# Yukun-Huang/DreamWaltz-G

Measured on AMD Instinct MI355X. Metric: SDS steps/sec @512^2, 100k Gaussians, SD1.5+ControlNet; raster Mpix/s vs HBM roofline, higher is better.
Workload: dtype f32x

## Files before the change

### dreamwaltz-g_amd/csrc/gemm.hip

```cpp
#include "dwg_common.h"
#include "dwg_prof_internal.h"
#include "../../include/dwg_gemm.h"
#include <cstdlib>
#include <type_traits>

#if defined(DWG_GEMM_X_TU)
#include "dwg_xfmt.h"
typedef _Float16 HT;
#define DWG_DTYPE_HALF DWG_DTYPE_F32X
#define DWG_MFMA16(a, b, c) __builtin_amdgcn_mfma_f32_32x32x16_f16(a, b, c, 0, 0, 0)
#define DWG_HALF_NAME "f32x"
#elif defined(DWG_GEMM_F16_TU)
typedef _Float16 HT;
#define DWG_DTYPE_HALF DWG_DTYPE_F16
#define DWG_MFMA16(a, b, c) __builtin_amdgcn_mfma_f32_32x32x16_f16(a, b, c, 0, 0, 0)
#define DWG_HALF_NAME "f16"
#else
typedef __bf16 HT;
#define DWG_DTYPE_HALF DWG_DTYPE_BF16
#define DWG_MFMA16(a, b, c) __builtin_amdgcn_mfma_f32_32x32x16_bf16(a, b, c, 0, 0, 0)
#define DWG_HALF_NAME "bf16"
#endif

namespace {

typedef __attribute__((ext_vector_type(8))) HT bf16x8;
typedef __attribute__((ext_vector_type(16))) float f32x16;

struct ConvP {
    int enabled, Cin, Hin, Win, Hout, Wout, KH, KW, stride, pad_t, pad_l, dil;
    int up;
    int cin1;
    const void* A2;
};

struct GemmP {
    const void* A; const void* B; void* C; const void* bias; const void* residual;
    int M, N, K;
    long long sam, sak, sbn, sbk, ldc, ldr;
    int nb2;
    long long bA1, bA2, bB1, bB2, bC1, bC2, bR1, bR2;
    int act; float alpha;
    int out_bf16, res_bf16, bias_per_row, splitk, accumulate;
    float* ws;
    int bias_row_div;
    long long bias_ld;
    ConvP conv;
};

__device__ __forceinline__ float bf2f(HT x) { return (float)x; }
__device__ __forceinline__ HT f2bf(float x) { return (HT)x; }

struct bf16x4_t { HT v[4]; };
#ifdef DWG_GEMM_X_TU
__device__ __forceinline__ float ld_half1(const void* base, long long i) { return dwg_x_get1(base, i); }
__device__ __forceinline__ void st_half1(void* base, long long i, float v) { dwg_x_put1(base, i, v); }
__device__ __forceinline__ void ld_half4(const void* base, long long i, float (&v)[4]) { dwg_x_get4(base, i, v); }
__device__ __forceinline__ void st_half4(void* base, long long i, const float (&v)[4]) { dwg_x_put4(base, i, v); }
#else
__device__ __forceinline__ float ld_half1(const void* base, long long i) { return bf2f(reinterpret_cast<const HT*>(base)[i]); }
__device__ __forceinline__ void st_half1(void* base, long long i, float v) { reinterpret_cast<HT*>(base)[i] = f2bf(v); }
__device__ __forceinline__ void ld_half4(const void* base, long long i, float (&v)[4]) {
    const bf16x4_t r = *reinterpret_cast<const bf16x4_t*>(reinterpret_cast<const HT*>(base) + i);
#pragma unroll
    for (int e = 0; e < 4; e++) v[e] = bf2f(r.v[e]);
}
__device__ __forceinline__ void st_half4(void* base, long long i, const float (&v)[4]) {
    bf16x4_t o;
#pragma unroll
    for (int e = 0; e < 4; e++) o.v[e] = f2bf(v[e]);
    *reinterpret_cast<bf16x4_t*>(reinterpret_cast<HT*>(base) + i) = o;
}
#endif

template <bool LIGHT = false>
__device__ __forceinline__ float apply_act(float v, int act) {
    if constexpr (LIGHT) return act == 3 ? v / (1.f + __expf(-v)) : v;
    switch (act) {
        case 1: return v > 0.f ? v : 0.f;
        case 2: return v > 0.f ? v : 0.01f * v;
        case 3: return v / (1.f + __expf(-v));
        case 4: return 0.5f * v * (1.f + erff(v * 0.70710678118654752f));
        case 5: return 1.f / (1.f + __expf(-v));
        default: return v;
    }
}

template <typename T> struct TT;
template <> struct TT<HT> { static constexpr int VEC = 8; static constexpr int BK = 64; static constexpr int PAD = 8; };
template <> struct TT<float> { static constexpr int VEC = 4; static constexpr int BK = 16; static constexpr int PAD = 4; };

enum { MODE_KVEC = 0, MODE_RVEC = 1, MODE_SCALAR = 2, MODE_CONV = 3 };

template <typename T, int VEC> struct Chunk { T v[VEC]; };

template <typename T, int VEC>
__device__ __forceinline__ Chunk<T, VEC> load_vec(const T* p) {
    Chunk<T, VEC> c;
    *reinterpret_cast<uint4*>(&c) = *reinterpret_cast<const uint4*>(p);
    return c;
}
template <typename T, int VEC>
__device__ __forceinline__ Chunk<T, VEC> zero_chunk() {
    Chunk<T, VEC> c;
    *reinterpret_cast<uint4*>(&c) = make_uint4(0u, 0u, 0u, 0u);
    return c;
}

template <typename T, int ROWS, int MODE>
struct TileLoader {
    static constexpr int VEC = TT<T>::VEC, BK = TT<T>::BK, LDT = BK + TT<T>::PAD;
    static constexpr int CPR = BK / VEC, RPI = 256 / CPR;
    static constexpr int CPK = ROWS / VEC, KPI = 256 / CPK;
    static constexpr int NCH = (MODE == MODE_SCALAR) ? (ROWS * BK / 256) : (MODE == MODE_RVEC ? BK / KPI : ROWS / RPI);
    Chunk<T, VEC> regs[(MODE == MODE_SCALAR) ? 1 : NCH];
    T sregs[(MODE == MODE_SCALAR) ? NCH : 1];
    const T* rowptr[(MODE == MODE_KVEC) ? NCH : 1];
    int iy0[(MODE == MODE_CONV) ? NCH : 1], ix0[(MODE == MODE_CONV) ? NCH : 1];
    long long pix0[(MODE == MODE_CONV) ? NCH : 1];
    bool rok[(MODE == MODE_CONV) ? NCH : 1];
    const T* base; long long srow, sk; int nrows, r0, kcur, kend;
    int ci, ky, kx;

    __device__ __forceinline__ void init(const T* base_, long long srow_, long long sk_, int nrows_, int r0_, int kbeg, int kend_,
                                         const ConvP& cv) {
        base = base_; srow = srow_; sk = sk_; nrows = nrows_; r0 = r0_; kend = kend_;
        const int tid = threadIdx.x;
        if (MODE == MODE_KVEC) {
            kcur = kbeg + (tid % CPR) * VEC;
#pragma unroll
            for (int i = 0; i < NCH; i++) {
                int r = r0 + tid / CPR + i * RPI;
                rowptr[i] = r < nrows ? base + (long long)r * srow : nullptr;
            }
        } else if (MODE == MODE_CONV) {
            kcur = kbeg + (tid % CPR) * VEC;
            const int hw = cv.Hout * cv.Wout;
#pragma unroll
            for (int i = 0; i < NCH; i++) {
                int r = r0 + tid / CPR + i * RPI;
                rok[i] = r < nrows;
                int rr = rok[i] ? r : 0;
                int img = rr / hw, rem = rr - img * hw;
                int oy = rem / cv.Wout, ox = rem - oy * cv.Wout;
                iy0[i] = oy * cv.stride - cv.pad_t; ix0[i] = ox * cv.stride - cv.pad_l;
                pix0[i] = (long long)img * cv.Hin * cv.Win;
            }
            int tap = kcur / cv.Cin;
            ci = kcur - tap * cv.Cin; ky = tap / cv.KW; kx = tap - ky * cv.KW;
        } else {
            kcur = kbeg;
        }
    }

    __device__ __forceinline__ void advance(const ConvP& cv) {
        kcur += BK;
        if (MODE == MODE_CONV) {
            ci += BK;
            while (ci >= cv.Cin) { ci -= cv.Cin; if (++kx == cv.KW) { kx = 0; ++ky; } }
        }
    }

    __device__ __forceinline__ void load(const ConvP& cv) {
        const int tid = threadIdx.x;
        if (MODE == MODE_KVEC) {
            const bool kok = kcur < kend;
#pragma unroll
            for (int i = 0; i < NCH; i++)
                regs[i] = (kok && rowptr[i]) ? load_vec<T, VEC>(rowptr[i] + kcur) : zero_chunk<T, VEC>();
        } else if (MODE == MODE_CONV) {
            const bool kok = kcur < kend;
            const T* src0 = ci < cv.cin1 ? base : reinterpret_cast<const T*>(cv.A2);
            const int cs = ci < cv.cin1 ? cv.cin1 : (cv.Cin - cv.cin1);
            const int co = ci < cv.cin1 ? ci : ci - cv.cin1;
#pragma unroll
            for (int i = 0; i < NCH; i++) {
                int iy = iy0[i] + ky, ix = ix0[i] + kx;
                bool ok = kok && rok[i] && iy >= 0 && ix >= 0;
                if (cv.dil > 1) { ok = ok && (iy % cv.dil == 0) && (ix % cv.dil == 0); iy /= cv.dil; ix /= cv.dil; }
                if (cv.up > 1) { iy >>= 1; ix >>= 1; }
                ok = ok && iy < cv.Hin && ix < cv.Win;
                regs[i] = ok ? load_vec<T, VEC>(src0 + (pix0[i] + (long long)iy * cv.Win + ix) * cs + co) : zero_chunk<T, VEC>();
            }
        } else if (MODE == MODE_RVEC) {
#pragma unroll
            for (int i = 0; i < NCH; i++) {
                int kk = tid / CPK + i * KPI, rc = tid % CPK;
                int r = r0 + rc * VEC, k = kcur + kk;
                regs[i] = (r < nrows && k < kend) ? load_vec<T, VEC>(base + (long long)k * sk + r) : zero_chunk<T, VEC>();
            }
        } else {
#pragma unroll
            for (int i = 0; i < NCH; i++) {
                int c = tid + i * 256, row = c / BK, kk = c - row * BK;
                int r = r0 + row, k = kcur + kk;
                sregs[i] = (r < nrows && k < kend) ? base[(long long)r * srow + (long long)k * sk] : (T)0.f;
            }
        }
    }

    __device__ __forceinline__ void store(T* lds) {
        const int tid = threadIdx.x;
        if (MODE == MODE_KVEC || MODE == MODE_CONV) {
#pragma unroll
            for (int i = 0; i < NCH; i++)
                *reinterpret_cast<uint4*>(lds + (tid / CPR + i * RPI) * LDT + (tid % CPR) * VEC) = *reinterpret_cast<uint4*>(&regs[i]);
        } else if (MODE == MODE_RVEC) {
#pragma unroll
            for (int i = 0; i < NCH; i++) {
                int kk = tid / CPK + i * KPI, rc = tid % CPK;
#pragma unroll
                for (int e = 0; e < VEC; e++) lds[(rc * VEC + e) * LDT + kk] = regs[i].v[e];
            }
        } else {
#pragma unroll
            for (int i = 0; i < NCH; i++) {
                int c = tid + i * 256, row = c / BK, kk = c - row * BK;
                lds[row * LDT + kk] = sregs[i];
            }
        }
    }
};

template <typename T>
__device__ __forceinline__ void mma_tile(const T* sa, const T* sb, int lane, f32x16& acc);

template <>
__device__ __forceinline__ void mma_tile<HT>(const HT* sa, const HT* sb, int lane, f32x16& acc) {
    constexpr int LDT = TT<HT>::BK + TT<HT>::PAD;
    const HT* pa = sa + (lane & 31) * LDT + (lane >> 5) * 8;
    const HT* pb = sb + (lane & 31) * LDT + (lane >> 5) * 8;
#pragma unroll
    for (int ks = 0; ks < TT<HT>::BK / 16; ks++) {
        bf16x8 a = *reinterpret_cast<const bf16x8*>(pa + ks * 16);
        bf16x8 b = *reinterpret_cast<const bf16x8*>(pb + ks * 16);
        acc = DWG_MFMA16(a, b, acc);
    }
}
template <>
__device__ __forceinline__ void mma_tile<float>(const float* sa, const float* sb, int lane, f32x16& acc) {
    constexpr int LDT = TT<float>::BK + TT<float>::PAD;
    const float* pa = sa + (lane & 31) * LDT + (lane >> 5);
    const float* pb = sb + (lane & 31) * LDT + (lane >> 5);
#pragma unroll
    for (int ks = 0; ks < TT<float>::BK / 2; ks++)
        acc = __builtin_amdgcn_mfma_f32_32x32x2f32(pa[ks * 2], pb[ks * 2], acc, 0, 0, 0);
}

template <bool LIGHT = false>
__device__ __forceinline__ void epilogue_store(const GemmP& p, float v, int row, int col, long long coff, long long roff) {
    const long long ci = coff + (long long)row * p.ldc + col;
    if (p.bias) v += reinterpret_cast<const float*>(p.bias)[p.bias_row_div > 0 ? (long long)(row / p.bias_row_div) * p.bias_ld + col
                                                                             : (p.bias_per_row ? row : col)];
    v = apply_act<LIGHT>(v, p.act);
    if (p.residual) {
        const long long ri = roff + (long long)row * p.ldr + col;
        v += p.res_bf16 ? ld_half1(p.residual, ri) : reinterpret_cast<const float*>(p.residual)[ri];
    }
    if (p.out_bf16) st_half1(p.C, ci, v);
    else if (p.accumulate) reinterpret_cast<float*>(p.C)[ci] += v;
    else reinterpret_cast<float*>(p.C)[ci] = v;
}

__device__ __forceinline__ bool epilogue_vec_ok(const GemmP& p, long long coff, long long roff) {
    bool ok = (p.N & 3) == 0 && (p.ldc & 3) == 0 && (coff & 3) == 0 && ((uintptr_t)p.C & 15) == 0;
    if (p.residual) ok = ok && (p.ldr & 3) == 0 && (roff & 3) == 0 && ((uintptr_t)p.residual & 15) == 0;
    return ok;
}

template <bool LIGHT = false>
__device__ __forceinline__ void epilogue_store4(const GemmP& p, float (&v)[4], int row, int col, long long coff, long long roff, bool vec_ok) {
    if (!vec_ok || col + 3 >= p.N) {
#pragma unroll
        for (int e = 0; e < 4; e++)
            if (col + e < p.N) epilogue_store<LIGHT>(p, v[e], row, col + e, coff, roff);
        return;
    }
    if (p.bias) {
        const float* b = reinterpret_cast<const float*>(p.bias);
        if (p.bias_row_div > 0) {
            b += (long long)(row / p.bias_row_div) * p.bias_ld + col;
            v[0] += b[0]; v[1] += b[1]; v[2] += b[2]; v[3] += b[3];
        } else if (p.bias_per_row) {
            const float br = b[row];
            v[0] += br; v[1] += br; v[2] += br; v[3] += br;
        } else {
            v[0] += b[col]; v[1] += b[col + 1]; v[2] += b[col + 2]; v[3] += b[col + 3];
        }
    }
#pragma unroll
    for (int e = 0; e < 4; e++) v[e] = apply_act<LIGHT>(v[e], p.act);
    if (p.residual) {
        const long long ri = roff + (long long)row * p.ldr + col;
        if (p.res_bf16) {
            float r[4];
            ld_half4(p.residual, ri, r);
#pragma unroll
            for (int e = 0; e < 4; e++) v[e] += r[e];
        } else {
            float4 r = *reinterpret_cast<const float4*>(reinterpret_cast<const float*>(p.residual) + ri);
            v[0] += r.x; v[1] += r.y; v[2] += r.z; v[3] += r.w;
        }
    }
    const long long ci = coff + (long long)row * p.ldc + col;
    if (p.out_bf16) {
        st_half4(p.C, ci, v);
    } else {
        float4* dst = reinterpret_cast<float4*>(reinterpret_cast<float*>(p.C) + ci);
        float4 o = make_float4(v[0], v[1], v[2], v[3]);
        if (p.accumulate) { float4 c = *dst; o.x += c.x; o.y += c.y; o.z += c.z; o.w += c.w; }
        *dst = o;
    }
}

template <int BN, int BM = 128> struct EpiLds {
    static constexpr int LDC = BN + 4;
    static constexpr int passes(size_t lds_bytes) {
        return lds_bytes >= (size_t)BM * LDC * 4 ? 1 : (lds_bytes >= (size_t)(BM / 2) * LDC * 4 ? 2 : 4);
    }
    static constexpr size_t bytes(int npass) { return (size_t)(BM / npass) * LDC * 4; }
};

template <int BN, int NPASS, int TM, int TN, bool LIGHT, int BM = 128, int NT = 256, typename RowFn>
__device__ __forceinline__ void tile_epilogue_lds(const GemmP& p, f32x16 (&acc)[TM][TN], float* sC, int n0, int wm, int wn, int lane, int tid,
                                                  int ks_id, long long coff, long long roff, RowFn row_of) {
    constexpr int LDC = EpiLds<BN, BM>::LDC, C4 = BN / 4, PR = BM / NPASS;
    constexpr int BPP = BM / 32 / NPASS;
    static_assert(NT % C4 == 0 && (C4 & (C4 - 1)) == 0, "a thread keeps one column group");
    const bool vec_ok = epilogue_vec_ok(p, coff, roff);
    const int lrow = lane & 31, lhalf = (lane >> 5) * 4;
    const bool geglu = p.act == 6;
    const float* bias = reinterpret_cast<const float*>(p.bias);
    const bool fast = vec_ok && !geglu && !p.accumulate && !p.bias_per_row && (p.splitk <= 1 || p.ws) &&
                      (!bias || p.bias_row_div > 0 || ((uintptr_t)bias & 15) == 0) &&
                      (!bias || p.bias_row_div <= 0 || (((uintptr_t)bias & 15) == 0 && (p.bias_ld & 3) == 0)) &&
                      (p.splitk <= 1 || ((uintptr_t)p.ws & 15) == 0);
#pragma unroll 1
    for (int q = 0; q < NPASS; q++) {
        __syncthreads();
#pragma unroll
        for (int i = 0; i < TM; i++) {
            const int rb = wm * TM + i;
            if (NPASS > 1 && rb / BPP != q) continue;
            float* dst = sC + ((NPASS > 1 ? rb % BPP : rb) * 32 + lrow) * LDC + wn * 64 + lhalf;
#pragma unroll
            for (int j = 0; j < TN; j++)
#pragma unroll
                for (int r4 = 0; r4 < 4; r4++)
                    *reinterpret_cast<float4*>(dst + j * 32 + 8 * r4) =
                        make_float4(acc[i][j][4 * r4], acc[i][j][4 * r4 + 1], acc[i][j][4 * r4 + 2], acc[i][j][4 * r4 + 3]);
        }
        __syncthreads();
        if (geglu) {
            constexpr int G = C4 / 2, RSTEP = NT / G;
            const int o4 = tid & (G - 1), rl0 = tid / G;
            const int b = o4 >> 3, w = (o4 & 7) * 4;
            const int colp = n0 + b * 64 + w;
            if (colp + 35 < p.N) {
                float bh[4] = {0.f, 0.f, 0.f, 0.f}, bg[4] = {0.f, 0.f, 0.f, 0.f};
                if (bias) {
#pragma unroll
                    for (int e = 0; e < 4; e++) { bh[e] = bias[colp + e]; bg[e] = bias[colp + 32 + e]; }
                }
                const bool vec_store = ((p.ldc | coff) & 3) == 0 && ((uintptr_t)p.C & 7) == 0;
#pragma unroll 2
                for (int rl = rl0; rl < PR; rl += RSTEP) {
                    const int row = row_of(q * PR + rl);
                    if (row < 0) continue;
                    const float4 h = *reinterpret_cast<const float4*>(sC + rl * LDC + b * 64 + w);
                    const float4 g = *reinterpret_cast<const float4*>(sC + rl * LDC + b * 64 + 32 + w);
                    const float hv[4] = {h.x, h.y, h.z, h.w}, gv[4] = {g.x, g.y, g.z, g.w};
                    float v[4];
#pragma unroll
                    for (int e = 0; e < 4; e++) {
                        const float a = fmaf(hv[e], p.alpha, bh[e]);
                        const float gg = fmaf(gv[e], p.alpha, bg[e]);
                        v[e] = a * 0.5f * gg * (1.f + dwg_erf_fast(gg * 0.70710678118654752f));
                    }
                    const long long ci = coff + (long long)row * p.ldc + (n0 + b * 64) / 2 + w;
                    if (p.out_bf16) {
                        if (vec_store) {
                            st_half4(p.C, ci, v);
                        } else {
#pragma unroll
                            for (int e = 0; e < 4; e++) st_half1(p.C, ci + e, v[e]);
                        }
                    } else {
#pragma unroll
                        for (int e = 0; e < 4; e++) reinterpret_cast<float*>(p.C)[ci + e] = v[e];
                    }
                }
            }
            continue;
        }
        if (fast) {
            constexpr int RSTEP = NT / C4;
            const int c4 = tid & (C4 - 1), rl0 = tid / C4;
            const int col = n0 + c4 * 4;
            if (col < p.N) {
                const bool col_bias = bias && p.bias_row_div <= 0;
                float4 bc = make_float4(0.f, 0.f, 0.f, 0.f);
                if (col_bias) bc = *reinterpret_cast<const float4*>(bias + col);
                const bool slab = p.splitk > 1;
#pragma unroll 2
                for (int rl = rl0; rl < PR; rl += RSTEP) {
                    const int row = row_of(q * PR + rl);
                    if (row < 0) continue;
                    const float4 a = *reinterpret_cast<const float4*>(sC + rl * LDC + c4 * 4);
                    float v[4] = {a.x * p.alpha, a.y * p.alpha, a.z * p.alpha, a.w * p.alpha};
                    if (slab) {
                        *reinterpret_cast<float4*>(p.ws + ((long long)ks_id * p.M + row) * p.N + col) = make_float4(v[0], v[1], v[2], v[3]);
                        continue;
                    }
                    if (col_bias) { v[0] += bc.x; v[1] += bc.y; v[2] += bc.z; v[3] += bc.w; }
                    else if (bias) {
                        const float4 b = *reinterpret_cast<const float4*>(bias + (long long)(row / p.bias_row_div) * p.bias_ld + col);
                        v[0] += b.x; v[1] += b.y; v[2] += b.z; v[3] += b.w;
                    }
                    if (p.act == 3) {
#pragma unroll
                        for (int e = 0; e < 4; e++) v[e] = v[e] / (1.f + __expf(-v[e]));
                    } else if (p.act != 0) {
#pragma unroll
                        for (int e = 0; e < 4; e++) v[e] = apply_act<LIGHT>(v[e], p.act);
                    }
                    if (p.residual) {
                        const long long ri = roff + (long long)row * p.ldr + col;
                        if (p.res_bf16) {
                            float r[4];
                            ld_half4(p.residual, ri, r);
#pragma unroll
                            for (int e = 0; e < 4; e++) v[e] += r[e];
                        } else {
                            const float4 r = *reinterpret_cast<const float4*>(reinterpret_cast<const float*>(p.residual) + ri);
                            v[0] += r.x; v[1] += r.y; v[2] += r.z; v[3] += r.w;
                        }
                    }
                    const long long ci = coff + (long long)row * p.ldc + col;
                    if (p.out_bf16) {
                        st_half4(p.C, ci, v);
                    } else {
                        *reinterpret_cast<float4*>(reinterpret_cast<float*>(p.C) + ci) = make_float4(v[0], v[1], v[2], v[3]);
                    }
                }
            }
            continue;
        }
#pragma unroll 1
        for (int idx = tid; idx < PR * C4; idx += NT) {
            const int rl = idx / C4, c4 = idx - rl * C4;
            const int row = row_of(q * PR + rl), col = n0 + c4 * 4;
            if (row < 0 || col >= p.N) continue;
            const float4 a = *reinterpret_cast<const float4*>(sC + rl * LDC + c4 * 4);
            float v[4] = {a.x * p.alpha, a.y * p.alpha, a.z * p.alpha, a.w * p.alpha};
            if (p.splitk > 1) {
                if (p.ws) {
                    float* dst = p.ws + ((long long)ks_id * p.M + row) * p.N + col;
                    if ((p.N & 3) == 0) *reinterpret_cast<float4*>(dst) = make_float4(v[0], v[1], v[2], v[3]);
                    else {
#pragma unroll
                        for (int e = 0; e < 4; e++) if (col + e < p.N) dst[e] = v[e];
                    }
                } else {
#pragma unroll
                    for (int e = 0; e < 4; e++)
                        if (col + e < p.N) atomicAdd(reinterpret_cast<float*>(p.C) + coff + (long long)row * p.ldc + col + e, v[e]);
                }
                continue;
            }
            epilogue_store4<LIGHT>(p, v, row, col, coff, roff, vec_ok);
        }
    }
}

__global__ __launch_bounds__(256) void k_splitk_epilogue(GemmP p) {
    const long long n = (long long)p.M * p.N;
    if ((p.N & 3) == 0) {
        const bool vec_ok = epilogue_vec_ok(p, 0, 0);
        const int N4 = p.N >> 2;
        const long long n4 = n >> 2;
        for (long long i = (long long)blockIdx.x * 256 + threadIdx.x; i < n4; i += (long long)gridDim.x * 256) {
            const unsigned iu = (unsigned)i;
            const int row = (int)(iu / (unsigned)N4), col = (int)(iu - (unsigned)row * (unsigned)N4) * 4;
            const float4* src = reinterpret_cast<const float4*>(p.ws) + i;
            float4 a = src[0];
            int sidx = 1;
            for (; sidx + 3 < p.splitk; sidx += 4) {
                const float4 u0 = src[(long long)sidx * n4], u1 = src[(long long)(sidx + 1) * n4], u2 = src[(long long)(sidx + 2) * n4],
                             u3 = src[(long long)(sidx + 3) * n4];
                a.x += u0.x; a.y += u0.y; a.z += u0.z; a.w += u0.w;
                a.x += u1.x; a.y += u1.y; a.z += u1.z; a.w += u1.w;
                a.x += u2.x; a.y += u2.y; a.z += u2.z; a.w += u2.w;
                a.x += u3.x; a.y += u3.y; a.z += u3.z; a.w += u3.w;
            }
            if (sidx + 1 < p.splitk) {
                const float4 u0 = src[(long long)sidx * n4], u1 = src[(long long)(sidx + 1) * n4];
                a.x += u0.x; a.y += u0.y; a.z += u0.z; a.w += u0.w;
                a.x += u1.x; a.y += u1.y; a.z += u1.z; a.w += u1.w;
                sidx += 2;
            }
            if (sidx < p.splitk) {
                const float4 u = src[(long long)sidx * n4];
                a.x += u.x; a.y += u.y; a.z += u.z; a.w += u.w;
            }
            float v[4] = {a.x, a.y, a.z, a.w};
            epilogue_store4(p, v, row, col, 0, 0, vec_ok);
        }
        return;
    }
    for (long long i = (long long)blockIdx.x * 256 + threadIdx.x; i < n; i += (long long)gridDim.x * 256) {
        float v = 0.f;
        for (int s = 0; s < p.splitk; s++) v += p.ws[(long long)s * n + i];
        int row = (int)(i / p.N), col = (int)(i - (long long)row * p.N);
        epilogue_store(p, v, row, col, 0, 0);
    }
}

static void launch_splitk_epilogue(const GemmP& p, hipStream_t stream) {
    if (!(p.splitk > 1 && p.ws)) return;
    long long n = (long long)p.M * p.N;
    if ((p.N & 3) == 0) n >>= 2;
    int blocks = (int)((n + 255) / 256); if (blocks > 2048) blocks = 2048;
    DWG_LAUNCH("splitk_epilogue", k_splitk_epilogue, dim3(blocks), dim3(256), 0, stream, p);
}
template <typename T, int BN, int AMODE, int BMODE>
__global__ __launch_bounds__(256, (sizeof(T) == 4 || BN == 64) ? 2 : 1) void k_gemm(GemmP p) {
    constexpr int BM = 128, BK = TT<T>::BK, LDT = BK + TT<T>::PAD;
    constexpr int WN = BN / 64;
    constexpr int WM = 4 / WN;
    constexpr int TM = BM / WM / 32;
    constexpr int TN = 2;
    extern __shared__ __attribute__((aligned(16))) unsigned char smem_raw[];
    T* sA = reinterpret_cast<T*>(smem_raw);
    T* sB = sA + 2 * BM * LDT;
    const int tid = threadIdx.x, lane = tid & 63, wave = tid >> 6;
    const int wm = wave / WN, wn = wave % WN;
    const int m0 = blockIdx.x * BM;
    const int ntn = (p.N + BN - 1) / BN;
    const int n0 = (blockIdx.y % ntn) * BN;
    const int ks_id = blockIdx.y / ntn;
    const int z = blockIdx.z, z1 = z / p.nb2, z2 = z - z1 * p.nb2;
    const T* A = reinterpret_cast<const T*>(p.A) + z1 * p.bA1 + z2 * p.bA2;
    const T* B = reinterpret_cast<const T*>(p.B) + z1 * p.bB1 + z2 * p.bB2;
    int kbeg = 0, kend = p.K;
    if (p.splitk > 1) {
        int per = ((p.K + p.splitk - 1) / p.splitk + BK - 1) / BK * BK;
        kbeg = ks_id * per; kend = min(p.K, kbeg + per);
    }
    f32x16 acc[TM][TN];
#pragma unroll
    for (int i = 0; i < TM; i++)
#pragma unroll
        for (int j = 0; j < TN; j++)
#pragma unroll
            for (int r = 0; r < 16; r++) acc[i][j][r] = 0.f;

    TileLoader<T, BM, AMODE> la;
    TileLoader<T, BN, BMODE> lb;
    la.init(A, p.sam, p.sak, p.M, m0, kbeg, kend, p.conv);
    lb.init(B, p.sbn, p.sbk, p.N, n0, kbeg, kend, p.conv);
    const int nk = kend > kbeg ? (kend - kbeg + BK - 1) / BK : 0;
    if (nk > 0) {
        la.load(p.conv); lb.load(p.conv);
        la.store(sA); lb.store(sB);
    }
    __syncthreads();
    for (int kt = 0; kt < nk; kt++) {
        const int cur = kt & 1;
        if (kt + 1 < nk) {
            la.advance(p.conv); lb.advance(p.conv);
            la.load(p.conv); lb.load(p.conv);
        }
        const T* a = sA + cur * BM * LDT + (wm * TM * 32) * LDT;
        const T* b = sB + cur * BN * LDT + (wn * 64) * LDT;
#pragma unroll
        for (int i = 0; i < TM; i++)
#pragma unroll
            for (int j = 0; j < TN; j++) mma_tile<T>(b + j * 32 * LDT, a + i * 32 * LDT, lane, acc[i][j]);
        if (kt + 1 < nk) { la.store(sA + (cur ^ 1) * BM * LDT); lb.store(sB + (cur ^ 1) * BN * LDT); }
        __syncthreads();
    }
    constexpr int NPASS = EpiLds<BN>::passes((size_t)2 * (BM + BN) * LDT * sizeof(T));
    static_assert((size_t)2 * (BM + BN) * LDT * sizeof(T) >= EpiLds<BN>::bytes(NPASS), "epilogue staging fits in the operand stages");
    tile_epilogue_lds<BN, NPASS, TM, TN, false>(p, acc, reinterpret_cast<float*>(smem_raw), n0, wm, wn, lane, tid, ks_id, z1 * p.bC1 + z2 * p.bC2,
                                         z1 * p.bR1 + z2 * p.bR2, [&](int rl) { const int r = m0 + rl; return r < p.M ? r : -1; });
}

__device__ __attribute__((aligned(16))) unsigned char g_zero16[16];

template <int ROWS, bool CONV, int NW = 4>
struct GldsLoader {
    static constexpr int NJ = ROWS / (8 * NW);
    const HT* rowptr[CONV ? 1 : NJ];
    int iy0[CONV ? NJ : 1], ix0[CONV ? NJ : 1];
    long long pix0[CONV ? NJ : 1];
    bool rok[CONV ? NJ : 1];
    const HT* base;
    int kc[2], kend, ci[2], ky[2], kx[2];

    __device__ __forceinline__ void init(const HT* base_, long long srow, int nrows, int r0, int kbeg, int kend_, const ConvP& cv) {
        static_assert(NJ % 2 == 0, "row-block parity must equal j parity");
        base = base_; kend = kend_;
        const int lane = threadIdx.x & 63, wave = threadIdx.x >> 6, sub = lane >> 3;
        const int lg0 = (lane & 7) ^ (sub >> 1);
        kc[0] = kbeg + lg0 * 8; kc[1] = kbeg + (lg0 ^ 4) * 8;
        if (!CONV) {
#pragma unroll
            for (int j = 0; j < NJ; j++) {
                int r = r0 + (wave * NJ + j) * 8 + sub;
                rowptr[j] = r < nrows ? base + (long long)r * srow : nullptr;
            }
        } else {
            const int hw = cv.Hout * cv.Wout;
#pragma unroll
            for (int j = 0; j < NJ; j++) {
                int r = r0 + (wave * NJ + j) * 8 + sub;
                rok[j] = r < nrows;
                int rr = rok[j] ? r : 0;
                int img = rr / hw, rem = rr - img * hw;
                int oy = rem / cv.Wout, ox = rem - oy * cv.Wout;
                iy0[j] = oy * cv.stride - cv.pad_t; ix0[j] = ox * cv.stride - cv.pad_l;
                pix0[j] = (long long)img * cv.Hin * cv.Win;
            }
#pragma unroll
            for (int q = 0; q < 2; q++) {
                int tap = kc[q] / cv.Cin;
                ci[q] = kc[q] - tap * cv.Cin; ky[q] = tap / cv.KW; kx[q] = tap - ky[q] * cv.KW;
            }
        }
    }
    __device__ __forceinline__ void advance(const ConvP& cv) {
        kc[0] += 64; kc[1] += 64;
        if (CONV) {
#pragma unroll
            for (int q = 0; q < 2; q++) {
                ci[q] += 64;
                while (ci[q] >= cv.Cin) { ci[q] -= cv.Cin; if (++kx[q] == cv.KW) { kx[q] = 0; ++ky[q]; } }
            }
        }
    }
    __device__ __forceinline__ void issue(unsigned char* lds_tile, const ConvP& cv) {
        const int wave = __builtin_amdgcn_readfirstlane(threadIdx.x >> 6);
        const HT* zero = reinterpret_cast<const HT*>(g_zero16);
        const HT* src0[2] = {base, base}; int cs[2] = {0, 0}, co[2] = {0, 0};
        bool kok[2];
#pragma unroll
        for (int q = 0; q < 2; q++) {
            kok[q] = kc[q] < kend;
            if (CONV) {
                src0[q] = ci[q] < cv.cin1 ? base : reinterpret_cast<const HT*>(cv.A2);
                cs[q] = ci[q] < cv.cin1 ? cv.cin1 : (cv.Cin - cv.cin1);
                co[q] = ci[q] < cv.cin1 ? ci[q] : ci[q] - cv.cin1;
            }
        }
#pragma unroll
        for (int j = 0; j < NJ; j++) {
            const int q = j & 1;
            const HT* src;
            if (!CONV) {
                src = (kok[q] && rowptr[j]) ? rowptr[j] + kc[q] : zero;
            } else {
                int iy = iy0[j] + ky[q], ix = ix0[j] + kx[q];
                bool ok = kok[q] && rok[j] && iy >= 0 && ix >= 0;
                if (cv.dil > 1) { ok = ok && (iy % cv.dil == 0) && (ix % cv.dil == 0); iy /= cv.dil; ix /= cv.dil; }
                if (cv.up > 1) { iy >>= 1; ix >>= 1; }
                ok = ok && iy < cv.Hin && ix < cv.Win;
                src = ok ? src0[q] + (pix0[j] + (long long)iy * cv.Win + ix) * cs[q] + co[q] : zero;
            }
            unsigned char* dst = lds_tile + ((wave * NJ + j) * 8) * 128;
            __builtin_amdgcn_global_load_lds((const __attribute__((address_space(1))) void*)src,
                                             (__attribute__((address_space(3))) void*)dst, 16, 0, 0);
        }
    }
};

template <int ROWS, int NW = 4, bool CAT = false>
struct GldsConvFast {
    static constexpr int NJ = ROWS / (8 * NW);
    const unsigned char* pb[NJ];
    const unsigned char* pb2[CAT ? NJ : 1];
    unsigned int mask[NJ];
    int kcur, kend, tap, ci, ky, kx;

    __device__ __forceinline__ void init(const HT* base, long long, int nrows, int r0, int kbeg, int kend_, const ConvP& cv) {
        static_assert(NJ % 2 == 0, "row-block parity must equal j parity");
        const int lane = threadIdx.x & 63, wave = threadIdx.x >> 6, sub = lane >> 3;
        const int lg0 = (lane & 7) ^ (sub >> 1);
        kcur = kbeg; kend = kend_;
        tap = kbeg / cv.Cin; ci = kbeg - tap * cv.Cin; ky = tap / cv.KW; kx = tap - ky * cv.KW;
        const int hw = cv.Hout * cv.Wout;
        const int cs1 = CAT ? cv.cin1 : cv.Cin;
#pragma unroll
        for (int j = 0; j < NJ; j++) {
            const int r = r0 + (wave * NJ + j) * 8 + sub;
            const bool rok = r < nrows;
            const int rr = rok ? r : 0;
            const int img = rr / hw, rem = rr - img * hw;
            const int oy = rem / cv.Wout, ox = rem - oy * cv.Wout;
            const int iy0 = oy * cv.stride - cv.pad_t, ix0 = ox * cv.stride - cv.pad_l;
            unsigned int m = 0;
            for (int t = 0, y = 0; y < cv.KH; y++)
                for (int x = 0; x < cv.KW; x++, t++) {
                    const int iy = iy0 + y, ix = ix0 + x;
                    if (rok && iy >= 0 && iy < cv.Hin && ix >= 0 && ix < cv.Win) m |= 1u << t;
                }
            mask[j] = m;
            const long long pix = ((long long)img * cv.Hin + iy0) * cv.Win + ix0;
            pb[j] = reinterpret_cast<const unsigned char*>(base) + (pix * cs1 + (lg0 ^ ((j & 1) << 2)) * 8) * 2;
            if (CAT) pb2[j] = reinterpret_cast<const unsigned char*>(cv.A2) + (pix * (cv.Cin - cv.cin1) + (lg0 ^ ((j & 1) << 2)) * 8) * 2;
        }
    }
    __device__ __forceinline__ void advance(const ConvP& cv) {
        kcur += 64; ci += 64;
        const int w = ci >= cv.Cin ? 1 : 0;
        ci = w ? 0 : ci; tap += w; kx += w;
        const int w2 = kx == cv.KW ? 1 : 0;
        kx = w2 ? 0 : kx; ky += w2;
    }
    __device__ __forceinline__ void issue(unsigned char* lds_tile, const ConvP& cv) {
        const int wave = __builtin_amdgcn_readfirstlane(threadIdx.x >> 6);
        const unsigned char* zero = g_zero16;
        const bool second = CAT && ci >= cv.cin1;
        const int cs = CAT ? (second ? cv.Cin - cv.cin1 : cv.cin1) : cv.Cin;
        const long long uoff = (((long long)ky * cv.Win + kx) * cs + (second ? ci - cv.cin1 : ci)) * 2;
        const unsigned int bit = kcur < kend ? (1u << tap) : 0u;
#pragma unroll
        for (int j = 0; j < NJ; j++) {
            const unsigned char* src = (mask[j] & bit) ? ((CAT && second) ? pb2[j] : pb[j]) + uoff : zero;
            unsigned char* dst = lds_tile + ((wave * NJ + j) * 8) * 128;
            __builtin_amdgcn_global_load_lds((const __attribute__((address_space(1))) void*)src,
                                             (__attribute__((address_space(3))) void*)dst, 16, 0, 0);
        }
    }
};

template <int N>
__device__ __forceinline__ void wait_vmcnt() {
    __builtin_amdgcn_s_waitcnt((N & 15) | ((N >> 4) << 14) | (7 << 4) | (15 << 8));
}

template <int BM, int AKIND, int NW = 4> struct ALoaderOf { typedef GldsLoader<BM, false, NW> type; };
template <int BM, int NW> struct ALoaderOf<BM, 1, NW> { typedef GldsLoader<BM, true, NW> type; };
template <int BM, int NW> struct ALoaderOf<BM, 2, NW> { typedef GldsConvFast<BM, NW, false> type; };
template <int BM, int NW> struct ALoaderOf<BM, 3, NW> { typedef GldsConvFast<BM, NW, true> type; };

template <int BM, int BN> struct GldsGeom {
    static constexpr int WN = BN / 64, WM = (BM == 128 && BN == 64) ? 4 : BM / 64, NW = WM * WN, NT = NW * 64, TM = BM / WM / 32, TN = 2;
};

template <int BM, int BN, int AKIND, int S>
__device__ __forceinline__ void gemm_glds_body(const GemmP& p) {
    typedef GldsGeom<BM, BN> Geo;
    constexpr int WN = Geo::WN, WM = Geo::WM, NW = Geo::NW, NT = Geo::NT, TM = Geo::TM, TN = Geo::TN;
    constexpr int ABYTES = BM * 128, BBYTES = BN * 128, STAGE = ABYTES + BBYTES;
    extern __shared__ __attribute__((aligned(16))) unsigned char smem_raw[];
    const int tid = threadIdx.x, lane = tid & 63, wave = tid >> 6;
    const int wm = wave / WN, wn = wave % WN;
    const int gm = (p.M + BM - 1) / BM, ntn = (p.N + BN - 1) / BN;
    const int nwg = gridDim.x;
    int id = blockIdx.x;
    {
        const int q = nwg / 8, r = nwg % 8, xcd = id % 8, loc = id / 8;
        id = (xcd < r ? xcd * (q + 1) : r * (q + 1) + (xcd - r) * q) + loc;
    }
    const int tile = id % (gm * ntn), ks_id = id / (gm * ntn);
    const int m0 = (tile / ntn) * BM, n0 = (tile % ntn) * BN;
    const int z = blockIdx.z, z1 = z / p.nb2, z2 = z - z1 * p.nb2;
    const HT* A = reinterpret_cast<const HT*>(p.A) + z1 * p.bA1 + z2 * p.bA2;
    const HT* B = reinterpret_cast<const HT*>(p.B) + z1 * p.bB1 + z2 * p.bB2;
    int kbeg = 0, kend = p.K;
    if (p.splitk > 1) {
        int per = ((p.K + p.splitk - 1) / p.splitk + 63) / 64 * 64;
        kbeg = ks_id * per; kend = min(p.K, kbeg + per);
    }
    f32x16 acc[TM][TN];
#pragma unroll
    for (int i = 0; i < TM; i++)
#pragma unroll
        for (int j = 0; j < TN; j++)
#pragma unroll
            for (int r = 0; r < 16; r++) acc[i][j][r] = 0.f;
#ifdef DWG_GEMM_X_TU
    f32x16 acx[TM][TN];
#pragma unroll
    for (int i = 0; i < TM; i++)
#pragma unroll
        for (int j = 0; j < TN; j++)
#pragma unroll
            for (int r = 0; r < 16; r++) acx[i][j][r] = 0.f;
#endif
    typename ALoaderOf<BM, AKIND, NW>::type la;
    GldsLoader<BN, false, NW> lb;
    la.init(A, p.sam, p.M, m0, kbeg, kend, p.conv);
    lb.init(B, p.sbn, p.N, n0, kbeg, kend, p.conv);
    const int nk = kend > kbeg ? (kend - kbeg + 63) / 64 : 0;
    constexpr int LPT = (BM + BN) * 128 / (NT * 16);
#pragma unroll
    for (int s = 0; s < S - 1; s++) {
        la.issue(smem_raw + s * STAGE, p.conv); lb.issue(smem_raw + s * STAGE + ABYTES, p.conv);
        la.advance(p.conv); lb.advance(p.conv);
    }
    const int frow = lane & 31, fx = (lane >> 1) & 7, fh = lane >> 5;
#ifdef DWG_GEMM_X_TU
    constexpr int KS = 2;
    struct Frag { bf16x8 ah[TM], al[TM], bh[TN], bl[TN]; };
#else
    constexpr int KS = 4;
    struct Frag { bf16x8 af[TM], bf[TN]; };
#endif
    auto load_frags = [&](int stage, int ks, Frag& f) {
        const unsigned char* ta = smem_raw + stage * STAGE + (wm * TM * 32 + frow) * 128;
        const unsigned char* tb = smem_raw + stage * STAGE + ABYTES + (wn * 64 + frow) * 128;
#ifdef DWG_GEMM_X_TU
        const int offh = (((ks * 4 + fh * 2) ^ fx) << 4), offl = (((ks * 4 + fh * 2 + 1) ^ fx) << 4);
#pragma unroll
        for (int i = 0; i < TM; i++) {
            f.ah[i] = *reinterpret_cast<const bf16x8*>(ta + i * 32 * 128 + offh);
            f.al[i] = *reinterpret_cast<const bf16x8*>(ta + i * 32 * 128 + offl);
        }
#pragma unroll
        for (int j = 0; j < TN; j++) {
            f.bh[j] = *reinterpret_cast<const bf16x8*>(tb + j * 32 * 128 + offh);
            f.bl[j] = *reinterpret_cast<const bf16x8*>(tb + j * 32 * 128 + offl);
        }
#else
        const int off = (((ks * 2 + fh) ^ fx) << 4);
#pragma unroll
        for (int i = 0; i < TM; i++) f.af[i] = *reinterpret_cast<const bf16x8*>(ta + i * 32 * 128 + off);
#pragma unroll
        for (int j = 0; j < TN; j++) f.bf[j] = *reinterpret_cast<const bf16x8*>(tb + j * 32 * 128 + off);
#endif
    };
    auto mma = [&](const Frag& f) {
#ifdef DWG_GEMM_X_TU
#pragma unroll
        for (int i = 0; i < TM; i++)
#pragma unroll
            for (int j = 0; j < TN; j++) acc[i][j] = DWG_MFMA16(f.bh[j], f.ah[i], acc[i][j]);
#pragma unroll
        for (int i = 0; i < TM; i++)
#pragma unroll
            for (int j = 0; j < TN; j++) acx[i][j] = DWG_MFMA16(f.bl[j], f.ah[i], acx[i][j]);
#pragma unroll
        for (int i = 0; i < TM; i++)
#pragma unroll
            for (int j = 0; j < TN; j++) acx[i][j] = DWG_MFMA16(f.bh[j], f.al[i], acx[i][j]);
#else
#pragma unroll
        for (int i = 0; i < TM; i++)
#pragma unroll
            for (int j = 0; j < TN; j++) acc[i][j] = DWG_MFMA16(f.bf[j], f.af[i], acc[i][j]);
#endif
    };
    auto wait_tile_and_lds = [&]() {
        constexpr int N = (S - 2) * LPT;
        __builtin_amdgcn_s_waitcnt((N & 15) | ((N >> 4) << 14) | (7 << 4) | (0 << 8));
    };
    Frag F[2];
    int cur = 0, nxt = S - 1;
    if (nk > 0) {
        wait_vmcnt<(S - 2) * LPT>();
        __builtin_amdgcn_s_barrier();
        load_frags(0, 0, F[0]);
        __builtin_amdgcn_s_waitcnt(0xC07F);
    }
#ifdef DWG_GEMM_X_TU
    constexpr int MPS = 3 * TM * TN;
#else
    constexpr int MPS = TM * TN;
#endif
    for (int kt = 0; kt < nk; kt++) {
        const int cnext = cur + 1 == S ? 0 : cur + 1;
#pragma unroll
        for (int ks = 0; ks < KS; ks++) {
            if (ks + 1 < KS) {
                load_frags(cur, ks + 1, F[(ks + 1) & 1]);
            } else {
                wait_tile_and_lds();
                __builtin_amdgcn_s_barrier();
                load_frags(cnext, 0, F[0]);
            }
            __builtin_amdgcn_sched_barrier(0);
            if (ks == 0) {
                la.issue(smem_raw + nxt * STAGE, p.conv); lb.issue(smem_raw + nxt * STAGE + ABYTES, p.conv);
                la.advance(p.conv); lb.advance(p.conv);
            }
            mma(F[ks & 1]);
            if (ks == 0) {
#pragma unroll
                for (int m = 0; m < MPS; m++) {
                    __builtin_amdgcn_sched_group_barrier(0x008, 1, 0);
                    __builtin_amdgcn_sched_group_barrier(0x006, (LPT * 10 + MPS - 1) / MPS, 0);
                    __builtin_amdgcn_sched_group_barrier(0x020, (LPT + MPS - 1) / MPS, 0);
                }
            }
            __builtin_amdgcn_sched_barrier(0);
        }
        __builtin_amdgcn_s_waitcnt(0xC07F);
        cur = cnext; nxt = nxt + 1 == S ? 0 : nxt + 1;
    }
    wait_vmcnt<0>();
#ifdef DWG_GEMM_X_TU
#pragma unroll
    for (int i = 0; i < TM; i++)
#pragma unroll
        for (int j = 0; j < TN; j++)
#pragma unroll
            for (int r = 0; r < 16; r++) acc[i][j][r] = fmaf(acx[i][j][r], DWG_X_LO_INV, acc[i][j][r]);
#endif
    constexpr int NPASS = EpiLds<BN, BM>::passes((size_t)S * STAGE);
    static_assert((size_t)S * STAGE >= EpiLds<BN, BM>::bytes(NPASS), "epilogue staging fits in the operand stages");
    tile_epilogue_lds<BN, NPASS, TM, TN, false, BM, NT>(p, acc, reinterpret_cast<float*>(smem_raw), n0, wm, wn, lane, tid, ks_id, z1 * p.bC1 + z2 * p.bC2,
                                         z1 * p.bR1 + z2 * p.bR2, [&](int rl) { const int r = m0 + rl; return r < p.M ? r : -1; });
}

template <int BN, int AKIND, int S>
__global__ __launch_bounds__(256, 2) void k_gemm_glds(GemmP p) {
    gemm_glds_body<128, BN, AKIND, S>(p);
}

template <int BM, int BN, int AKIND, int S>
__global__ __launch_bounds__(512, 2) void k_gemm_glds8(GemmP p) {
    static_assert(GldsGeom<BM, BN>::NT == 512, "eight waves");
    gemm_glds_body<BM, BN, AKIND, S>(p);
}

static double gemm_flops(const GemmP& p, int batch) {
    double f = 2.0 * p.M * p.N * p.K * batch;
#ifdef DWG_GEMM_X_TU
    f *= 0.5;
#endif
    if (p.conv.enabled && p.conv.dil > 1) f /= (double)(p.conv.dil * p.conv.dil);
    return f;
}

template <int BN, int AKIND>
static void launch_glds(const GemmP& p, int batch, hipStream_t stream, const char* name) {
    constexpr int S = (BN == 64 && AKIND != 1) ? 3 : 2;
    size_t lds = (size_t)S * (128 + BN) * 128;
    static bool attr_set = false;
    if (!attr_set) {
        hipFuncSetAttribute(reinterpret_cast<const void*>(&k_gemm_glds<BN, AKIND, S>), hipFuncAttributeMaxDynamicSharedMemorySize, (int)lds);
        attr_set = true;
    }
    dim3 grid(((p.M + 127) / 128) * ((p.N + BN - 1) / BN) * (p.splitk > 1 ? p.splitk : 1), 1, batch);
    static const char* const sym[2][4] = {{"k_gemm_glds<64, 0, 3>", "k_gemm_glds<64, 1, 2>", "k_gemm_glds<64, 2, 3>", "k_gemm_glds<64, 3, 3>"},
                                          {"k_gemm_glds<128, 0, 2>", "k_gemm_glds<128, 1, 2>", "k_gemm_glds<128, 2, 2>", "k_gemm_glds<128, 3, 2>"}};
    DWG_LAUNCH_W(name, sym[BN == 128][AKIND], gemm_flops(p, batch), (k_gemm_glds<BN, AKIND, S>), grid, dim3(256), lds, stream, p);
    launch_splitk_epilogue(p, stream);
}

template <int BM, int BN, int AKIND>
static void launch_glds8(const GemmP& p, int batch, hipStream_t stream, const char* name) {
    constexpr int S = 3;
    const size_t lds = (size_t)S * (BM + BN) * 128;
    static bool attr_set = false;
    if (!attr_set) {
        hipFuncSetAttribute(reinterpret_cast<const void*>(&k_gemm_glds8<BM, BN, AKIND, S>), hipFuncAttributeMaxDynamicSharedMemorySize, (int)lds);
        attr_set = true;
    }
    dim3 grid(((p.M + BM - 1) / BM) * ((p.N + BN - 1) / BN) * (p.splitk > 1 ? p.splitk : 1), 1, batch);
    static const char* const sym[2][4] = {
        {"k_gemm_glds8<256, 128, 0, 3>", "k_gemm_glds8<256, 128, 1, 3>", "k_gemm_glds8<256, 128, 2, 3>", "k_gemm_glds8<256, 128, 3, 3>"},
        {"k_gemm_glds8<128, 256, 0, 3>", "k_gemm_glds8<128, 256, 1, 3>", "k_gemm_glds8<128, 256, 2, 3>", "k_gemm_glds8<128, 256, 3, 3>"}};
    DWG_LAUNCH_W(name, sym[BN == 256][AKIND], gemm_flops(p, batch), (k_gemm_glds8<BM, BN, AKIND, S>), grid, dim3(512), lds, stream, p);
    launch_splitk_epilogue(p, stream);
}

template <bool V> struct BoolC { static constexpr bool value = V; };
template <int BN, int NW> struct Patch2Geom {
    static constexpr int PH = NW == 8 ? 16 : 8, PW = 16, HP = PH + 2, WP = PW + 2, NPIX = HP * WP, BM = PH * PW;
    static constexpr int NPI = (NPIX + 7) / 8;
    static constexpr int PPW = (NPI + NW - 1) / NW;
    static constexpr int WN = BN / 64, WM = NW / WN, TM = BM / WM / 32, TN = 2, NT = NW * 64;
    static constexpr int NJW = BN / (8 * NW);
    static constexpr int PBYTES = NPI * 8 * 128, BBYTES = BN * 128;
};

template <int BN, bool SPLIT, int NW, int NBS>
__global__ __launch_bounds__(NW * 64, 2) void k_conv3x3_patch2(GemmP p) {
    typedef Patch2Geom<BN, NW> G;
    constexpr int PH = G::PH, PW = G::PW, WP = G::WP, NPIX = G::NPIX, NPI = G::NPI, PPW = G::PPW;
    constexpr int WN = G::WN, WM = G::WM, TM = G::TM, TN = G::TN, NT = G::NT, NJW = G::NJW, BM = G::BM;
    constexpr int PBYTES = G::PBYTES, BBYTES = G::BBYTES;
    static_assert(NJW >= 1 && (NJW % 2 == 0 || NJW == 1), "row-block parity");
    extern __shared__ __attribute__((aligned(16))) unsigned char smem_raw[];
    unsigned char* sP = smem_raw;
    unsigned char* sB = smem_raw + 2 * PBYTES;
    const ConvP& cv = p.conv;
    const int tid = threadIdx.x, lane = tid & 63, wave = tid >> 6;
    const int wv = __builtin_amdgcn_readfirstlane(wave);
    const int wm = wave / WN, wn = wave % WN;
    const int tiles_x = (cv.Wout + PW - 1) / PW, tiles_y = (cv.Hout + PH - 1) / PH;
    const int nimg = p.M / (cv.Hout * cv.Wout);
    const int gm = nimg * tiles_y * tiles_x, ntn = (p.N + BN - 1) / BN;
    int id = blockIdx.x;
    {
        const int nwg = gridDim.x, q = nwg / 8, r = nwg % 8, xcd = id % 8, loc = id / 8;
        id = (xcd < r ? xcd * (q + 1) : r * (q + 1) + (xcd - r) * q) + loc;
    }
    int ks_id = 0;
    if constexpr (SPLIT) { ks_id = id / (gm * ntn); id -= ks_id * gm * ntn; }
    const int mt = id / ntn, n0 = (id % ntn) * BN;
    const int img = mt / (tiles_y * tiles_x), trem = mt % (tiles_y * tiles_x);
    const int y0 = (trem / tiles_x) * PH, x0 = (trem % tiles_x) * PW;
    const HT* X = reinterpret_cast<const HT*>(p.A) + (long long)img * cv.Hin * cv.Win * cv.Cin;
    const HT* Wt = reinterpret_cast<const HT*>(p.B);
    const HT* zero = reinterpret_cast<const HT*>(g_zero16);
    const int sub = lane >> 3, lg0 = (lane & 7) ^ (sub >> 1);

    auto issue_patch = [&](int cc, bool valid, unsigned char* dst) {
#pragma unroll
        for (int q = 0; q < PPW; q++) {
            int inst = wv + q * NW;
            if (inst >= NPI) inst -= NW;
            const int pi = inst * 8 + sub;
            const int py = pi / WP, px = pi - py * WP;
            const int iy = y0 - 1 + py, ix = x0 - 1 + px;
            const bool ok = valid && pi < NPIX && iy >= 0 && iy < cv.Hin && ix >= 0 && ix < cv.Win;
            const HT* src = ok ? X + ((long long)iy * cv.Win + ix) * cv.Cin + (lg0 ^ ((inst & 1) << 2)) * 8 + cc * 64 : zero;
            __builtin_amdgcn_global_load_lds((const __attribute__((address_space(1))) void*)src,
                                             (__attribute__((address_space(3))) void*)(dst + inst * 8 * 128), 16, 0, 0);
        }
    };
    const HT* wrow[NJW];
#pragma unroll
    for (int j = 0; j < NJW; j++) {
        const int r = n0 + (wv * NJW + j) * 8 + sub;
        wrow[j] = r < p.N ? Wt + (long long)r * p.sbn + (lg0 ^ (((wv * NJW + j) & 1) << 2)) * 8 : nullptr;
    }
    auto issue_w = [&](int cc, int tap, bool valid, unsigned char* dst) {
        const long long kofs = (long long)tap * cv.Cin + cc * 64;
#pragma unroll
        for (int j = 0; j < NJW; j++) {
            const HT* src = (valid && wrow[j]) ? wrow[j] + kofs : zero;
            __builtin_amdgcn_global_load_lds((const __attribute__((address_space(1))) void*)src,
                                             (__attribute__((address_space(3))) void*)(dst + (wv * NJW + j) * 8 * 128), 16, 0, 0);
        }
    };
    f32x16 acc[TM][TN];
#pragma unroll
    for (int i = 0; i < TM; i++)
#pragma unroll
        for (int j = 0; j < TN; j++)
#pragma unroll
            for (int r = 0; r < 16; r++) acc[i][j][r] = 0.f;
#ifdef DWG_GEMM_X_TU
    f32x16 acx[TM][TN];
#pragma unroll
    for (int i = 0; i < TM; i++)
#pragma unroll
        for (int j = 0; j < TN; j++)
#pragma unroll
            for (int r = 0; r < 16; r++) acx[i][j][r] = 0.f;
    constexpr int KS = 2, MPS = 3 * TM * TN;
    struct Frag { bf16x8 ah[TM], al[TM], bh[TN], bl[TN]; };
#else
    constexpr int KS = 4, MPS = TM * TN;
    struct Frag { bf16x8 af[TM], bf[TN]; };
#endif
    int pbase[TM];
#pragma unroll
    for (int i = 0; i < TM; i++) {
        const int r = (wm * TM + i) * 32 + (lane & 31);
        pbase[i] = (r / PW) * WP + (r % PW);
    }
    int cc0 = 0, ncc = cv.Cin / 64;
    if constexpr (SPLIT) {
        const int per = (ncc + p.splitk - 1) / p.splitk;
        cc0 = ks_id * per; ncc = min(ncc, cc0 + per);
    }
    const int frow = lane & 31, fx = (lane >> 1) & 7, fh = lane >> 5;
    const int nsteps = max(0, ncc - cc0) * 9;
    auto load_frags = [&](const unsigned char* pa, int toff, const unsigned char* tbs, int ks, Frag& f) {
        const unsigned char* tb = tbs + (wn * 64 + frow) * 128;
#ifdef DWG_GEMM_X_TU
        const int cl = ks * 4 + fh * 2;
#pragma unroll
        for (int i = 0; i < TM; i++) {
            const int pi = pbase[i] + toff, sw = (pi >> 1) & 7;
            f.ah[i] = *reinterpret_cast<const bf16x8*>(pa + pi * 128 + ((cl ^ sw) << 4));
            f.al[i] = *reinterpret_cast<const bf16x8*>(pa + pi * 128 + (((cl + 1) ^ sw) << 4));
        }
#pragma unroll
        for (int j = 0; j < TN; j++) {
            f.bh[j] = *reinterpret_cast<const bf16x8*>(tb + j * 32 * 128 + ((cl ^ fx) << 4));
            f.bl[j] = *reinterpret_cast<const bf16x8*>(tb + j * 32 * 128 + (((cl + 1) ^ fx) << 4));
        }
#else
        const int cl = ks * 2 + fh;
#pragma unroll
        for (int i = 0; i < TM; i++) {
            const int pi = pbase[i] + toff;
            f.af[i] = *reinterpret_cast<const bf16x8*>(pa + pi * 128 + ((cl ^ ((pi >> 1) & 7)) << 4));
        }
#pragma unroll
        for (int j = 0; j < TN; j++) f.bf[j] = *reinterpret_cast<const bf16x8*>(tb + j * 32 * 128 + ((cl ^ fx) << 4));
#endif
    };
    auto mma = [&](const Frag& f) {
#ifdef DWG_GEMM_X_TU
#pragma unroll
        for (int i = 0; i < TM; i++)
#pragma unroll
            for (int j = 0; j < TN; j++) acc[i][j] = DWG_MFMA16(f.bh[j], f.ah[i], acc[i][j]);
#pragma unroll
        for (int i = 0; i < TM; i++)
#pragma unroll
            for (int j = 0; j < TN; j++) acx[i][j] = DWG_MFMA16(f.bl[j], f.ah[i], acx[i][j]);
#pragma unroll
        for (int i = 0; i < TM; i++)
#pragma unroll
            for (int j = 0; j < TN; j++) acx[i][j] = DWG_MFMA16(f.bh[j], f.al[i], acx[i][j]);
#else
#pragma unroll
        for (int i = 0; i < TM; i++)
#pragma unroll
            for (int j = 0; j < TN; j++) acc[i][j] = DWG_MFMA16(f.bf[j], f.af[i], acc[i][j]);
#endif
    };
    issue_patch(cc0, nsteps > 0, sP + (cc0 & 1) * PBYTES);
#pragma unroll
    for (int g = 0; g < NBS - 1; g++) issue_w(cc0 + g / 9, g % 9, g < nsteps, sB + g * BBYTES);
    Frag F[2];
    if (nsteps > 0) {
        wait_vmcnt<(NBS - 2) * NJW>();
        __builtin_amdgcn_s_barrier();
        load_frags(sP + (cc0 & 1) * PBYTES, 0, sB, 0, F[0]);
        __builtin_amdgcn_s_waitcnt(0xC07F);
    }
    int bst = 0;
    auto step = [&](auto is_tap0, int tap, int cc, const unsigned char* pa, const unsigned char* pan) {
        constexpr bool TAP0 = decltype(is_tap0)::value;
        const int ty = tap >= 6 ? 2 : (tap >= 3 ? 1 : 0);
        const int toff = ty * WP + (tap - 3 * ty);
        const int bnext = bst + 1 == NBS ? 0 : bst + 1;
        const int bfill = bst == 0 ? NBS - 1 : bst - 1;
        const unsigned char* tb = sB + bst * BBYTES;
#pragma unroll
        for (int ks = 0; ks < KS; ks++) {
            if (ks + 1 < KS) {
                load_frags(pa, toff, tb, ks + 1, F[(ks + 1) & 1]);
            } else {
                if (TAP0 || tap <= NBS - 2) {
                    constexpr int N = (NBS - 2) * NJW + PPW;
                    __builtin_amdgcn_s_waitcnt((N & 15) | ((N >> 4) << 14) | (7 << 4) | (0 << 8));
                } else {
                    constexpr int N = (NBS - 2) * NJW;
                    __builtin_amdgcn_s_waitcnt((N & 15) | ((N >> 4) << 14) | (7 << 4) | (0 << 8));
                }
                __builtin_amdgcn_s_barrier();
                const int ntap = tap == 8 ? 0 : tap + 1;
                const int nty = ntap >= 6 ? 2 : (ntap >= 3 ? 1 : 0);
                load_frags(tap == 8 ? pan : pa, nty * WP + (ntap - 3 * nty), sB + bnext * BBYTES, 0, F[0]);
            }
            __builtin_amdgcn_sched_barrier(0);
            if (ks == 0) {
                const int ft = tap + NBS - 1, fcc = cc + (ft >= 9 ? 1 : 0), ftap = ft >= 9 ? ft - 9 : ft;
                issue_w(fcc, ftap, fcc < ncc, sB + bfill * BBYTES);
                if (TAP0) issue_patch(cc + 1, cc + 1 < ncc, const_cast<unsigned char*>(pan));
            }
            mma(F[ks & 1]);
            if (ks == 0) {
                constexpr int NL = NJW + (TAP0 ? PPW : 0);
#pragma unroll
                for (int m = 0; m < MPS; m++) {
                    __builtin_amdgcn_sched_group_barrier(0x008, 1, 0);
                    __builtin_amdgcn_sched_group_barrier(0x006, (NL * 8 + MPS - 1) / MPS, 0);
                    __builtin_amdgcn_sched_group_barrier(0x020, (NL + MPS - 1) / MPS, 0);
                }
            }
            __builtin_amdgcn_sched_barrier(0);
        }
        __builtin_amdgcn_s_waitcnt(0xC07F);
        bst = bnext;
    };
    for (int cc = cc0; cc < ncc; cc++) {
        const unsigned char* pa = sP + (cc & 1) * PBYTES;
        const unsigned char* pan = sP + ((cc + 1) & 1) * PBYTES;
        step(BoolC<true>{}, 0, cc, pa, pan);
#pragma unroll 1
        for (int tap = 1; tap < 9; tap++) step(BoolC<false>{}, tap, cc, pa, pan);
    }
    wait_vmcnt<0>();
    __builtin_amdgcn_s_barrier();
#ifdef DWG_GEMM_X_TU
#pragma unroll
    for (int i = 0; i < TM; i++)
#pragma unroll
        for (int j = 0; j < TN; j++)
#pragma unroll
            for (int r = 0; r < 16; r++) acc[i][j][r] = fmaf(acx[i][j][r], DWG_X_LO_INV, acc[i][j][r]);
#endif
    constexpr int NPASS = EpiLds<BN, BM>::passes((size_t)2 * PBYTES + NBS * BBYTES);
    static_assert((size_t)2 * PBYTES + NBS * BBYTES >= EpiLds<BN, BM>::bytes(NPASS), "epilogue staging fits in the patch / weight buffers");
    tile_epilogue_lds<BN, NPASS, TM, TN, !SPLIT, BM, NT>(p, acc, reinterpret_cast<float*>(smem_raw), n0, wm, wn, lane, tid, ks_id, 0, 0, [&](int rr) {
        const int y = y0 + rr / PW, x = x0 + rr % PW;
        return (y < cv.Hout && x < cv.Wout) ? (img * cv.Hout + y) * cv.Wout + x : -1;
    });
}

template <int BN, int NW, int NBS>
static void launch_conv3x3_patch2(const GemmP& p, hipStream_t stream, const char* name) {
    typedef Patch2Geom<BN, NW> G;
    const size_t lds = (size_t)2 * G::PBYTES + (size_t)NBS * G::BBYTES;
    const ConvP& cv = p.conv;
    const int nimg = p.M / (cv.Hout * cv.Wout);
    const int gm = nimg * ((cv.Hout + G::PH - 1) / G::PH) * ((cv.Wout + G::PW - 1) / G::PW);
    dim3 grid(gm * ((p.N + BN - 1) / BN) * (p.splitk > 1 ? p.splitk : 1));
    static bool attr_set = false;
    if (!attr_set) {
        hipFuncSetAttribute(reinterpret_cast<const void*>(&k_conv3x3_patch2<BN, false, NW, NBS>), hipFuncAttributeMaxDynamicSharedMemorySize, (int)lds);
        hipFuncSetAttribute(reinterpret_cast<const void*>(&k_conv3x3_patch2<BN, true, NW, NBS>), hipFuncAttributeMaxDynamicSharedMemorySize, (int)lds);
        attr_set = true;
    }
    static_assert((NW == 8 && BN == 128 && NBS == 4) || (NW == 4 && BN == 64 && NBS == 4) || (NW == 4 && BN == 128 && NBS == 2), "symbol table below");
    const char* sym = NW == 8 ? (p.splitk > 1 && p.ws ? "k_conv3x3_patch2<128, true, 8, 4>" : "k_conv3x3_patch2<128, false, 8, 4>")
                              : (BN == 64 ? (p.splitk > 1 && p.ws ? "k_conv3x3_patch2<64, true, 4, 4>" : "k_conv3x3_patch2<64, false, 4, 4>")
                                          : (p.splitk > 1 && p.ws ? "k_conv3x3_patch2<128, true, 4, 2>" : "k_conv3x3_patch2<128, false, 4, 2>"));
    if (p.splitk > 1 && p.ws)
        DWG_LAUNCH_W(name, sym, gemm_flops(p, 1), (k_conv3x3_patch2<BN, true, NW, NBS>), grid, dim3(NW * 64), lds, stream, p);
    else
        DWG_LAUNCH_W(name, sym, gemm_flops(p, 1), (k_conv3x3_patch2<BN, false, NW, NBS>), grid, dim3(NW * 64), lds, stream, p);
    launch_splitk_epilogue(p, stream);
}

template <typename T, int BN, int AMODE, int BMODE>
static void launch(const GemmP& p, int batch, hipStream_t stream, const char* name) {
    constexpr int LDT = TT<T>::BK + TT<T>::PAD;
    size_t lds = (size_t)2 * (128 + BN) * LDT * sizeof(T);
    dim3 grid((p.M + 127) / 128, ((p.N + BN - 1) / BN) * (p.splitk > 1 ? p.splitk : 1), batch);
    static bool attr_set = false;
    if (!attr_set) {
        hipFuncSetAttribute(reinterpret_cast<const void*>(&k_gemm<T, BN, AMODE, BMODE>), hipFuncAttributeMaxDynamicSharedMemorySize,
                            (int)lds);
        attr_set = true;
    }
    DWG_LAUNCH_W(name, (sizeof(T) == 2 ? "k_gemm<" DWG_HALF_NAME ">" : "k_gemm<f32>"), gemm_flops(p, batch), (k_gemm<T, BN, AMODE, BMODE>), grid,
                 dim3(256), lds, stream, p);
    launch_splitk_epilogue(p, stream);
}

template <typename T, int BN, int AMODE>
static void dispatch_b(const GemmP& p, int bmode, int batch, hipStream_t s, const char* name) {
    if (bmode == MODE_KVEC) launch<T, BN, AMODE, MODE_KVEC>(p, batch, s, name);
    else if (bmode == MODE_RVEC) launch<T, BN, AMODE, MODE_RVEC>(p, batch, s, name);
    else launch<T, BN, AMODE, MODE_SCALAR>(p, batch, s, name);
}
template <typename T, int BN>
static void dispatch_a(const GemmP& p, int amode, int bmode, int batch, hipStream_t s, const char* name) {
    if (amode == MODE_KVEC) dispatch_b<T, BN, MODE_KVEC>(p, bmode, batch, s, name);
    else if (amode == MODE_RVEC) dispatch_b<T, BN, MODE_RVEC>(p, bmode, batch, s, name);
    else if (amode == MODE_CONV) dispatch_b<T, BN, MODE_CONV>(p, bmode, batch, s, name);
    else dispatch_b<T, BN, MODE_SCALAR>(p, bmode, batch, s, name);
}

static int batch_of(const dwg_gemm_desc* d) { return d->batch1 * d->batch2; }

static int tile_bn(const dwg_gemm_desc* d) {
    if (d->N <= 64) return 64;
    const long long blocks128 = (long long)((d->M + 127) / 128) * ((d->N + 127) / 128) * batch_of(d);
    return blocks128 < 256 ? 64 : 128;
}

constexpr int kCUs = 256, kMinWgs = 200;
static bool fills_cus(long long wgs) {
    const long long rounds = (wgs + kCUs - 1) / kCUs;
    return wgs >= kMinWgs && wgs * 100 >= rounds * kCUs * 80;
}

constexpr int kSplitkTarget = 256;
constexpr int kSplitkNoSplit = 384;
constexpr int kSplitkMinSteps = 12;
static int auto_splitk(int M, int N, int K, int bn, int bk) {
    long long blocks = (long long)((M + 127) / 128) * ((N + bn - 1) / bn);
    if (blocks >= kSplitkNoSplit || K < 2 * kSplitkMinSteps * bk) return 1;
    if (2.0 * M * N * K < 4.0e8) return 1;
    long long sk = kSplitkTarget / blocks;
    long long kmax = K / (kSplitkMinSteps * bk);
    if (sk > kmax) sk = kmax;
    if (sk > 16) sk = 16;
    return sk >= 2 ? (int)sk : 1;
}

constexpr int kBigMinK = 1280, kBigMaxTiles = 2048;
constexpr int kBigMinSteps = 8, kBigSkMax = 24;
static int big_tile(int M, int N, int K, int* splitk_out) {
    *splitk_out = 1;
    if (K < kBigMinK) return 0;
    int bm = 0;
    if (M >= 192) { if (N >= 128 && (N % 128 == 0 || N >= 640)) bm = 256; }
    else if (N >= 256) bm = 128;
    if (!bm) return 0;
    const int bn = bm == 256 ? 128 : 256;
    const long long tiles = (long long)((M + bm - 1) / bm) * ((N + bn - 1) / bn);
    if (tiles > kBigMaxTiles) return 0;
    long long sk = 1;
    if (tiles < kCUs) {
        sk = kCUs / tiles;
        const long long kmax = K / (kBigMinSteps * 64);
        if (sk > kmax) sk = kmax;
        if (sk > kBigSkMax) sk = kBigSkMax;
        if (sk < 1) sk = 1;
    }
    if (!fills_cus(tiles * sk)) return 0;
    *splitk_out = (int)sk;
    return bm;
}

template <typename T>
static int pick_mode(const void* base, long long srow, long long sk, int nrows, int K, const long long* boffs, int nboffs) {
    constexpr int VEC = TT<T>::VEC;
    bool aligned = ((uintptr_t)base % 16) == 0;
    for (int i = 0; i < nboffs; i++) aligned = aligned && (boffs[i] % VEC == 0);
    if (sk == 1 && aligned && K % VEC == 0 && srow % VEC == 0) return MODE_KVEC;
    if (srow == 1 && aligned && nrows % VEC == 0 && sk % VEC == 0) return MODE_RVEC;
    return MODE_SCALAR;
}

static int splitk_of(const dwg_gemm_desc* d) {
    if (d->splitk > 1) return d->splitk;
    if (d->splitk != 0 || d->act == DWG_ACT_GEGLU_PAIR) return 1;
    return auto_splitk(d->M, d->N, d->K, tile_bn(d), d->dtype == DWG_DTYPE_HALF ? TT<HT>::BK : TT<float>::BK);
}
static bool slabs_possible(const dwg_gemm_desc* d) { return batch_of(d) == 1 && (long long)d->M * d->N < (1LL << 33); }
static long long fit_workspace(const dwg_gemm_desc* d, long long sk) {
    while (sk > 1 && (size_t)sk * d->M * d->N * sizeof(float) > d->workspace_bytes) sk--;
    return sk;
}

enum Family { FAM_GENERIC, FAM_GLDS, FAM_GLDS8, FAM_PATCH2 };
struct Plan {
    Family fam;
    int bm, bn, nw;
    int amode, bmode;
    int akind;
    int splitk;
    bool slabs;
};

constexpr int kPatchMinM = 8192;
constexpr int kPatch8MinSteps = 100;

static int make_plan(const dwg_gemm_desc* d, const GemmP& p, Plan& pl) {
    const bool half = d->dtype == DWG_DTYPE_HALF;
#if defined(DWG_GEMM_F16_TU) || defined(DWG_GEMM_X_TU)
    if (!half) return DWG_E_ARG;
#endif
    pl = Plan{FAM_GENERIC, 128, tile_bn(d), 4, MODE_KVEC, MODE_KVEC, 0, d->splitk > 1 ? d->splitk : 1, false};
    if (d->workspace && slabs_possible(d)) {
        pl.splitk = (int)fit_workspace(d, splitk_of(d));
        pl.slabs = pl.splitk > 1;
    }
    const long long ao[2] = {p.bA1, p.bA2}, bo[2] = {p.bB1, p.bB2};
    if (p.conv.enabled) {
        const int vec = half ? TT<HT>::VEC : TT<float>::VEC;
        if (d->conv_cin % vec != 0 || ((uintptr_t)d->A % 16) != 0) return DWG_E_ARG;
        if (d->A2 && (d->conv_cin1 % vec != 0 || d->conv_cin1 <= 0 || d->conv_cin1 >= d->conv_cin || ((uintptr_t)d->A2 % 16) != 0))
            return DWG_E_ARG;
        if (d->K != d->conv_kh * d->conv_kw * d->conv_cin) return DWG_E_ARG;
        pl.amode = MODE_CONV;
    } else {
        pl.amode = half ? pick_mode<HT>(p.A, p.sam, p.sak, p.M, p.K, ao, 2) : pick_mode<float>(p.A, p.sam, p.sak, p.M, p.K, ao, 2);
    }
    pl.bmode = half ? pick_mode<HT>(p.B, p.sbn, p.sbk, p.N, p.K, bo, 2) : pick_mode<float>(p.B, p.sbn, p.sbk, p.N, p.K, bo, 2);
    if (!half) return DWG_OK;
    if (pl.bmode != MODE_KVEC || (pl.amode != MODE_KVEC && pl.amode != MODE_CONV)) {
#ifdef DWG_GEMM_X_TU
        return DWG_E_ARG;
#else
        return DWG_OK;
#endif
    }
    const ConvP& cv = p.conv;
    const char* minm = getenv("DWG_CONV_PATCH_MINM");
    const int patch_min_m = minm ? atoi(minm) : kPatchMinM;
    const bool patch_geom = pl.amode == MODE_CONV && batch_of(d) == 1 && d->conv_kh == 3 && d->conv_kw == 3 && d->conv_stride == 1 &&
                            cv.dil == 1 && cv.up == 1 && d->conv_pad_t == 1 && d->conv_pad_l == 1 && !d->A2 && d->conv_cin % 64 == 0 &&
                            d->conv_hout == d->conv_hin && d->conv_wout == d->conv_win && d->conv_wout >= 16 && d->conv_hout >= 8;
    const int ncc = d->conv_cin / 64;
    if (patch_geom && d->splitk <= 1 && d->conv_hout % 16 == 0 && d->conv_wout % 16 == 0 && (d->N % 128 == 0 || d->N >= 512)) {
        const long long tiles8 = (long long)(d->M / 256) * ((d->N + 127) / 128);
        long long sk = 1;
        if (tiles8 < kMinWgs && d->workspace && d->splitk == 0 && slabs_possible(d)) {
            sk = kCUs / tiles8;
            if (sk > ncc / 2) sk = ncc / 2;
            sk = fit_workspace(d, sk);
            if (sk < 1) sk = 1;
            const long long per = (ncc + sk - 1) / sk;
            sk = (ncc + per - 1) / per;
        }
        const long long steps = (ncc + sk - 1) / sk * 9;
        const bool worth = sk > 1 || steps >= kPatch8MinSteps || d->M < patch_min_m;
        if (worth && fills_cus(tiles8 * sk) && (d->act == 0 || d->act == 3 || sk > 1)) {
            pl = Plan{FAM_PATCH2, 256, 128, 8, MODE_CONV, pl.bmode, 0, (int)sk, sk > 1};
            return DWG_OK;
        }
    }
    if (patch_geom && d->M >= patch_min_m && (d->act == 0 || d->act == 3 || pl.splitk > 1)) {
        if (pl.splitk > 1) {
            const int gm = (d->M / (d->conv_hout * d->conv_wout)) * ((d->conv_hout + 7) / 8) * ((d->conv_wout + 15) / 16);
            const int blocks = gm * ((d->N + pl.bn - 1) / pl.bn);
            int sk = blocks >= 256 ? 1 : (384 + blocks - 1) / blocks;
            if (sk > ncc / 2) sk = ncc / 2;
            if (sk > pl.splitk) sk = pl.splitk;
            if (sk < 2) sk = 1;
            pl.splitk = sk;
            pl.slabs = pl.slabs && sk > 1;
        }
        pl.fam = FAM_PATCH2;
        return DWG_OK;
    }
    const bool fast_geom = pl.amode == MODE_CONV && d->conv_cin % 64 == 0 && cv.dil == 1 && cv.up == 1 && d->conv_kh * d->conv_kw <= 32;
    const bool cat_fast = d->A2 && d->conv_cin1 % 64 == 0 && (d->conv_cin - d->conv_cin1) % 64 == 0;
    pl.akind = pl.amode != MODE_CONV ? 0 : (fast_geom && !d->A2 ? 2 : (fast_geom && cat_fast ? 3 : 1));
    int big_sk = 1;
    const int big_bm = d->splitk <= 1 ? big_tile(d->M, d->N, d->K, &big_sk) : 0;
    if (big_bm) {
        if (d->act == DWG_ACT_GEGLU_PAIR || !d->workspace || !slabs_possible(d) || d->splitk == 1) big_sk = 1;
        big_sk = (int)fit_workspace(d, big_sk);
        const int bbn = big_bm == 256 ? 128 : 256;
        const long long tiles = (long long)((d->M + big_bm - 1) / big_bm) * ((d->N + bbn - 1) / bbn) * batch_of(d);
        if (fills_cus(tiles * big_sk)) {
            pl = Plan{FAM_GLDS8, big_bm, bbn, 8, pl.amode, pl.bmode, pl.akind, big_sk, big_sk > 1};
            return DWG_OK;
        }
    }
    pl.fam = FAM_GLDS;
    return DWG_OK;
}

template <typename T>
static void launch_generic(const GemmP& p, const Plan& pl, int batch, hipStream_t s, const char* name) {
    if (pl.bn == 64) dispatch_a<T, 64>(p, pl.amode, pl.bmode, batch, s, name);
    else dispatch_a<T, 128>(p, pl.amode, pl.bmode, batch, s, name);
}
template <typename F>
static void with_akind(int akind, F f) {
    if (akind == 3) f(std::integral_constant<int, 3>{});
    else if (akind == 2) f(std::integral_constant<int, 2>{});
    else if (akind == 1) f(std::integral_constant<int, 1>{});
    else f(std::integral_constant<int, 0>{});
}

}

#ifdef DWG_GEMM_X_TU
static bool x_physical(const dwg_gemm_desc* d, dwg_gemm_desc* o) {
    if (!d) return false;
    *o = *d;
    if (d->dtype != DWG_DTYPE_F32X) return false;
    if (d->K % 8 || d->a_k_stride != 1 || d->b_k_stride != 1) return false;
    if ((d->a_row_stride | d->b_row_stride | d->a_batch1_stride | d->a_batch2_stride | d->b_batch1_stride | d->b_batch2_stride) % 8) return false;
    if (d->out_dtype == DWG_DTYPE_F32X && ((d->ldc | d->c_batch1_stride | d->c_batch2_stride) % 8 || ((uintptr_t)d->C % 16))) return false;
    if (d->residual && d->residual_dtype == DWG_DTYPE_F32X &&
        (((d->ldr ? d->ldr : d->ldc) | d->r_batch1_stride | d->r_batch2_stride) % 8 || ((uintptr_t)d->residual % 16))) return false;
    if (d->act == DWG_ACT_GEGLU_PAIR && d->out_dtype == DWG_DTYPE_F32X && d->N % 16) return false;
    if (d->conv_enabled && (d->conv_cin % 8 || (d->A2 && d->conv_cin1 % 8))) return false;
    o->K = 2 * d->K;
    o->a_row_stride = 2 * d->a_row_stride; o->b_row_stride = 2 * d->b_row_stride;
    o->a_batch1_stride = 2 * d->a_batch1_stride; o->a_batch2_stride = 2 * d->a_batch2_stride;
    o->b_batch1_stride = 2 * d->b_batch1_stride; o->b_batch2_stride = 2 * d->b_batch2_stride;
    o->conv_cin = 2 * d->conv_cin; o->conv_cin1 = 2 * d->conv_cin1;
    return true;
}
#endif

extern "C" {

#if defined(DWG_GEMM_X_TU)
#define DWG_GEMM_FN dwg_gemm_x
#define DWG_GEMM_WS_FN dwg_gemm_workspace_bytes_x
#elif defined(DWG_GEMM_F16_TU)
#define DWG_GEMM_FN dwg_gemm_f16
#define DWG_GEMM_WS_FN dwg_gemm_workspace_bytes_f16
#else
#define DWG_GEMM_FN dwg_gemm
#define DWG_GEMM_WS_FN dwg_gemm_workspace_bytes
size_t dwg_gemm_workspace_bytes_f16(const dwg_gemm_desc* d);
int dwg_gemm_f16(const dwg_gemm_desc* d, dwg_stream_t stream);
size_t dwg_gemm_workspace_bytes_x(const dwg_gemm_desc* d);
int dwg_gemm_x(const dwg_gemm_desc* d, dwg_stream_t stream);
#endif

size_t DWG_GEMM_WS_FN(const dwg_gemm_desc* d) {
#if !defined(DWG_GEMM_F16_TU) && !defined(DWG_GEMM_X_TU)
    if (d && d->dtype == DWG_DTYPE_F16) return dwg_gemm_workspace_bytes_f16(d);
    if (d && d->dtype == DWG_DTYPE_F32X) return dwg_gemm_workspace_bytes_x(d);
#endif
#ifdef DWG_GEMM_X_TU
    dwg_gemm_desc xd;
    if (!x_physical(d, &xd)) return 0;
    d = &xd;
#endif
    if (!d || d->M <= 0 || d->N <= 0 || !slabs_possible(d)) return 0;
    dwg_gemm_desc pd = *d;
    if (d->plan_m > d->M) pd.M = d->plan_m;
    d = &pd;
    int sk = splitk_of(d);
    if (d->dtype == DWG_DTYPE_HALF && d->splitk == 0 && d->act != DWG_ACT_GEGLU_PAIR) {
        int bsk = 1;
        if (big_tile(d->M, d->N, d->K, &bsk) && bsk > sk) sk = bsk;
    }
    return sk > 1 ? (size_t)sk * d->M * d->N * sizeof(float) : 0;
}

int DWG_GEMM_FN(const dwg_gemm_desc* d, dwg_stream_t stream_) {
#if !defined(DWG_GEMM_F16_TU) && !defined(DWG_GEMM_X_TU)
    if (d && d->dtype == DWG_DTYPE_F16) return dwg_gemm_f16(d, stream_);
    if (d && d->dtype == DWG_DTYPE_F32X) return dwg_gemm_x(d, stream_);
#endif
#ifdef DWG_GEMM_X_TU
    dwg_gemm_desc xd;
    if (!x_physical(d, &xd)) return DWG_E_ARG;
    d = &xd;
#endif
    if (!d || !d->A || !d->B || !d->C) return DWG_E_ARG;
    if (d->M < 0 || d->N < 0 || d->K < 0 || d->batch1 < 1 || d->batch2 < 1 || d->plan_m < 0) return DWG_E_ARG;
    if (d->M == 0 || d->N == 0) return DWG_OK;
    if (d->dtype != DWG_DTYPE_F32 && d->dtype != DWG_DTYPE_HALF) return DWG_E_ARG;
    if (d->splitk > 1 && !d->workspace && (d->out_dtype != DWG_DTYPE_F32 || d->bias || d->residual || d->act)) return DWG_E_ARG;
    if (d->accumulate && d->out_dtype != DWG_DTYPE_F32) return DWG_E_ARG;
    if (d->act == DWG_ACT_GEGLU_PAIR && (d->N % 64 != 0 || d->residual || d->splitk > 1 || d->bias_per_row || d->bias_row_div)) return DWG_E_ARG;
    if ((uintptr_t)d->workspace & 15) return DWG_E_ARG;
    GemmP p;
    p.A = d->A; p.B = d->B; p.C = d->C; p.bias = d->bias; p.residual = d->residual;
    p.M = d->M; p.N = d->N; p.K = d->K;
    p.sam = d->a_row_stride; p.sak = d->a_k_stride; p.sbn = d->b_row_stride; p.sbk = d->b_k_stride;
    p.ldc = d->ldc; p.ldr = d->ldr ? d->ldr : d->ldc;
    p.nb2 = d->batch2;
    p.bA1 = d->a_batch1_stride; p.bA2 = d->a_batch2_stride; p.bB1 = d->b_batch1_stride; p.bB2 = d->b_batch2_stride;
    p.bC1 = d->c_batch1_stride; p.bC2 = d->c_batch2_stride; p.bR1 = d->r_batch1_stride; p.bR2 = d->r_batch2_stride;
    p.act = d->act; p.alpha = d->alpha;
    p.out_bf16 = d->out_dtype == DWG_DTYPE_HALF; p.res_bf16 = d->residual_dtype == DWG_DTYPE_HALF;
    p.bias_per_row = d->bias_per_row; p.accumulate = d->accumulate;
    const bool plain1x1 = d->conv_enabled && d->conv_kh == 1 && d->conv_kw == 1 && d->conv_stride == 1 && d->conv_pad_t == 0 &&
                          d->conv_pad_l == 0 && d->conv_in_dilation <= 1 && d->conv_in_upsample <= 1 && !d->A2 && d->conv_hout == d->conv_hin &&
                          d->conv_wout == d->conv_win && d->K == d->conv_cin && batch_of(d) == 1;
    if (plain1x1) { p.sam = d->conv_cin; p.sak = 1; }
    p.conv.enabled = d->conv_enabled && !plain1x1;
    p.conv.Cin = d->conv_cin; p.conv.Hin = d->conv_hin; p.conv.Win = d->conv_win; p.conv.Hout = d->conv_hout;
    p.conv.Wout = d->conv_wout; p.conv.KH = d->conv_kh; p.conv.KW = d->conv_kw; p.conv.stride = d->conv_stride;
    p.conv.pad_t = d->conv_pad_t; p.conv.pad_l = d->conv_pad_l; p.conv.dil = d->conv_in_dilation > 1 ? d->conv_in_dilation : 1;
    p.conv.up = d->conv_in_upsample > 1 ? d->conv_in_upsample : 1;
    p.conv.A2 = d->A2; p.conv.cin1 = d->A2 ? d->conv_cin1 : d->conv_cin;
    p.bias_row_div = d->bias_row_div; p.bias_ld = d->bias_ld > 0 ? d->bias_ld : d->N;
    Plan pl;
    dwg_gemm_desc pd = *d;
    if (d->plan_m > d->M) pd.M = d->plan_m;
    const int rc = make_plan(&pd, p, pl);
    if (rc != DWG_OK) return rc;
    p.splitk = pl.splitk;
    p.ws = pl.slabs ? reinterpret_cast<float*>(d->workspace) : nullptr;
    const int batch = batch_of(d);
    hipStream_t stream = (hipStream_t)stream_;
    const char* name = d->name ? d->name : (d->conv_enabled ? "conv_igemm" : "gemm");
    switch (pl.fam) {
        case FAM_PATCH2:
            if (pl.nw == 8) launch_conv3x3_patch2<128, 8, 4>(p, stream, name);
            else if (pl.bn == 64) launch_conv3x3_patch2<64, 4, 4>(p, stream, name);
            else launch_conv3x3_patch2<128, 4, 2>(p, stream, name);
            break;
        case FAM_GLDS8:
            with_akind(pl.akind, [&](auto ak) {
                if (pl.bm == 256) launch_glds8<256, 128, decltype(ak)::value>(p, batch, stream, name);
                else launch_glds8<128, 256, decltype(ak)::value>(p, batch, stream, name);
            });
            break;
        case FAM_GLDS:
            with_akind(pl.akind, [&](auto ak) {
                if (pl.bn == 64) launch_glds<64, decltype(ak)::value>(p, batch, stream, name);
                else launch_glds<128, decltype(ak)::value>(p, batch, stream, name);
            });
            break;
        case FAM_GENERIC:
#if defined(DWG_GEMM_X_TU)
            return DWG_E_ARG;
#elif defined(DWG_GEMM_F16_TU)
            launch_generic<HT>(p, pl, batch, stream, name);
#else
            if (d->dtype == DWG_DTYPE_HALF) launch_generic<HT>(p, pl, batch, stream, name);
            else launch_generic<float>(p, pl, batch, stream, name);
#endif
            break;
    }
    DWG_RETURN_IF_LAUNCH_FAILED();
    return DWG_OK;
}

}
```

### dreamwaltz-g_amd/gemm.py

```python
import ctypes

import torch

from . import _lib

F32, BF16, F16, F32X = 0, 1, 2, 3
ACT = {None: 0, "none": 0, "relu": 1, "leaky_relu": 2, "silu": 3, "gelu": 4, "sigmoid": 5, "geglu_pair": 6}


class GemmDesc(ctypes.Structure):
    _fields_ = [
        ("A", ctypes.c_void_p), ("B", ctypes.c_void_p), ("C", ctypes.c_void_p), ("bias", ctypes.c_void_p),
        ("residual", ctypes.c_void_p),
        ("M", ctypes.c_int32), ("N", ctypes.c_int32), ("K", ctypes.c_int32),
        ("a_row_stride", ctypes.c_int64), ("a_k_stride", ctypes.c_int64), ("b_row_stride", ctypes.c_int64),
        ("b_k_stride", ctypes.c_int64), ("ldc", ctypes.c_int64), ("ldr", ctypes.c_int64),
        ("batch1", ctypes.c_int32), ("batch2", ctypes.c_int32),
        ("a_batch1_stride", ctypes.c_int64), ("a_batch2_stride", ctypes.c_int64), ("b_batch1_stride", ctypes.c_int64),
        ("b_batch2_stride", ctypes.c_int64), ("c_batch1_stride", ctypes.c_int64), ("c_batch2_stride", ctypes.c_int64),
        ("r_batch1_stride", ctypes.c_int64), ("r_batch2_stride", ctypes.c_int64),
        ("dtype", ctypes.c_int32), ("out_dtype", ctypes.c_int32), ("residual_dtype", ctypes.c_int32),
        ("act", ctypes.c_int32), ("alpha", ctypes.c_float), ("bias_per_row", ctypes.c_int32),
        ("splitk", ctypes.c_int32), ("accumulate", ctypes.c_int32),
        ("conv_enabled", ctypes.c_int32), ("conv_cin", ctypes.c_int32), ("conv_hin", ctypes.c_int32),
        ("conv_win", ctypes.c_int32), ("conv_hout", ctypes.c_int32), ("conv_wout", ctypes.c_int32),
        ("conv_kh", ctypes.c_int32), ("conv_kw", ctypes.c_int32), ("conv_stride", ctypes.c_int32),
        ("conv_pad_t", ctypes.c_int32), ("conv_pad_l", ctypes.c_int32), ("conv_in_dilation", ctypes.c_int32),
        ("conv_in_upsample", ctypes.c_int32), ("A2", ctypes.c_void_p), ("conv_cin1", ctypes.c_int32),
        ("bias_row_div", ctypes.c_int32), ("bias_ld", ctypes.c_int64),
        ("workspace", ctypes.c_void_p), ("workspace_bytes", ctypes.c_size_t),
        ("name", ctypes.c_char_p), ("plan_m", ctypes.c_int32),
    ]


def _dt(t):
    if t.dtype == torch.float32:
        return F32
    if t.dtype == torch.bfloat16:
        return BF16
    if t.dtype == torch.float16:
        return F16
    if t.dtype == torch.int32:
        return F32X
    raise TypeError("dwg gemm supports float32, bfloat16, float16 and f32x (int32-typed, xfmt.py) tensors, got %s" % t.dtype)


def _stream(t):
    return ctypes.c_void_p(torch.cuda.current_stream(t.device).cuda_stream)


def gemm_raw(A, B, C, M, N, K, a_strides, b_strides, ldc, bias=None, residual=None, ldr=0, act=None, alpha=1.0,
             batch=(1, 1), a_batch=(0, 0), b_batch=(0, 0), c_batch=(0, 0), r_batch=(0, 0), bias_per_row=False, splitk=1,
             accumulate=False, conv=None, name=None, conv_upsample=1, A2=None, cin1=0, bias_row_div=0, bias_ld=0, plan_m=0, run=True):
    if not A.is_cuda:
        raise RuntimeError("dreamwaltz_g_amd GEMM runs on the GPU only (HIP kernels)")
    d = GemmDesc()
    d.A, d.B, d.C = A.data_ptr(), B.data_ptr(), C.data_ptr()
    d.bias = bias.data_ptr() if bias is not None else None
    d.residual = residual.data_ptr() if residual is not None else None
    d.M, d.N, d.K = M, N, K
    d.a_row_stride, d.a_k_stride = a_strides
    d.b_row_stride, d.b_k_stride = b_strides
    d.ldc, d.ldr = ldc, ldr
    d.batch1, d.batch2 = batch
    d.a_batch1_stride, d.a_batch2_stride = a_batch
    d.b_batch1_stride, d.b_batch2_stride = b_batch
    d.c_batch1_stride, d.c_batch2_stride = c_batch
    d.r_batch1_stride, d.r_batch2_stride = r_batch
    d.dtype = _dt(A)
    assert _dt(B) == d.dtype, "A and B must share a dtype"
    d.out_dtype = _dt(C)
    d.residual_dtype = _dt(residual) if residual is not None else F32
    d.act = ACT[act]
    d.alpha = alpha
    d.bias_per_row = int(bias_per_row)
    d.splitk = splitk
    d.accumulate = int(accumulate)
    if conv is not None:
        d.conv_enabled = 1
        (d.conv_cin, d.conv_hin, d.conv_win, d.conv_hout, d.conv_wout, d.conv_kh, d.conv_kw, d.conv_stride, d.conv_pad_t,
         d.conv_pad_l, d.conv_in_dilation) = conv
    d.conv_in_upsample = conv_upsample
    if A2 is not None:
        d.A2 = A2.data_ptr(); d.conv_cin1 = cin1
    d.bias_row_div = bias_row_div
    d.bias_ld = bias_ld
    d.name = name.encode() if name else None
    d.plan_m = plan_m
    if not run:
        return d
    _lib.check(_lib.lib().dwg_gemm(ctypes.byref(d), _stream(A)), "dwg_gemm")
    return C


def run_desc(d, stream):
    rc = _lib.lib().dwg_gemm(ctypes.byref(d), stream)
    if rc != 0:
        raise RuntimeError("dwg_gemm failed with DWG error %d" % rc)


def linear(x, w, bias=None, act=None, out_dtype=None, residual=None, out=None, name=None):
    K = x.shape[-1]
    x2 = x.reshape(-1, K)
    M, N = x2.shape[0], w.shape[0]
    out_dtype = out_dtype or x.dtype
    y = out if out is not None else torch.empty(M, N, device=x.device, dtype=out_dtype)
    r2 = None if residual is None else residual.reshape(M, N)
    gemm_raw(x2, w, y, M, N, K, (x2.stride(0), x2.stride(1)), (w.stride(0), w.stride(1)), y.stride(0), bias=bias, residual=r2,
             ldr=0 if r2 is None else r2.stride(0), act=act, name=name)
    return y.reshape(*x.shape[:-1], N)


def conv2d_nhwc(x, w, bias=None, stride=1, pad=(1, 1), act=None, residual=None, out_hw=None, in_dilation=1, out_dtype=None,
                name=None):
    Bn, H, W, Cin = x.shape
    Cout, KH, KW, _ = w.shape
    Hv, Wv = (H - 1) * in_dilation + 1, (W - 1) * in_dilation + 1
    if out_hw is None:
        Ho = (Hv + 2 * pad[0] - KH) // stride + 1
        Wo = (Wv + 2 * pad[1] - KW) // stride + 1
    else:
        Ho, Wo = out_hw
    y = torch.empty(Bn, Ho, Wo, Cout, device=x.device, dtype=out_dtype or x.dtype)
    M, N, K = Bn * Ho * Wo, Cout, KH * KW * Cin
    gemm_raw(x, w, y, M, N, K, (0, 1), (K, 1), Cout, bias=bias, residual=residual, ldr=Cout if residual is not None else 0,
             act=act, conv=(Cin, H, W, Ho, Wo, KH, KW, stride, pad[0], pad[1], in_dilation), name=name)
    return y
```

### dreamwaltz-g_amd/sd15.py

```python
import ctypes
import os
import math
from collections import OrderedDict
from dataclasses import dataclass
from typing import Dict, List, Optional, Tuple

import torch

from . import _lib, gemm, xfmt

BF16 = torch.bfloat16

TORCH_DTYPE = {"bf16": torch.bfloat16, "f32": torch.float32, "f16": torch.float16, "f32x": xfmt.DTYPE}
DT_CODE = {"f32": 0, "bf16": 1, "f16": 2, "f32x": 3}


def dtype_name(dtype) -> str:
    names = {"bf16": "bf16", "bfloat16": "bf16", torch.bfloat16: "bf16", "f32": "f32", "fp32": "f32", "float32": "f32", torch.float32: "f32",
             "f16": "f16", "fp16": "f16", "float16": "f16", "half": "f16", torch.float16: "f16", "f32x": "f32x", "fp32x": "f32x"}
    if dtype not in names:
        raise ValueError("plan dtype must be one of bf16 / f32 / f16 / f32x, got %r" % (dtype,))
    return names[dtype]


@dataclass
class UNetConfig:
    in_channels: int = 4
    out_channels: int = 4
    block_out_channels: Tuple[int, ...] = (320, 640, 1280, 1280)
    layers_per_block: int = 2
    heads: int = 8
    cross_dim: int = 768
    groups: int = 32
    attn_blocks: Tuple[bool, ...] = (True, True, True, False)
    cond_channels: Tuple[int, ...] = (16, 32, 96, 256)
    cond_in_channels: int = 3

    @property
    def temb_dim(self):
        return self.block_out_channels[0] * 4


@dataclass
class VAEConfig:
    in_channels: int = 3
    block_out_channels: Tuple[int, ...] = (128, 256, 512, 512)
    layers_per_block: int = 2
    latent_channels: int = 4
    groups: int = 32
    scaling_factor: float = 0.18215


def _cfg_get(config, key, default):
    if config is None:
        return default
    if isinstance(config, dict):
        return config.get(key, default)
    return getattr(config, key, default)


def unet_config_from(config) -> "UNetConfig":
    d = UNetConfig()
    if config is None:
        return d
    boc = tuple(int(c) for c in _cfg_get(config, "block_out_channels", d.block_out_channels))
    down = tuple(_cfg_get(config, "down_block_types", ("CrossAttnDownBlock2D",) * 3 + ("DownBlock2D",)))
    heads = _cfg_get(config, "attention_head_dim", d.heads)
    if isinstance(heads, (list, tuple)):
        if len(set(heads)) != 1:
            raise NotImplementedError("per-level attention_head_dim %r (SDXL-style UNets are outside this path)" % (heads,))
        heads = heads[0]
    for key, want in (("transformer_layers_per_block", 1), ("class_embed_type", None), ("addition_embed_type", None), ("use_linear_projection", False),
                      ("only_cross_attention", False), ("dual_cross_attention", False)):
        got = _cfg_get(config, key, want)
        if got != want:
            raise NotImplementedError("UNet config %s=%r (SD-1.x layer graph only)" % (key, got))
    return UNetConfig(in_channels=int(_cfg_get(config, "in_channels", d.in_channels)), out_channels=int(_cfg_get(config, "out_channels", d.out_channels)),
                      block_out_channels=boc, layers_per_block=int(_cfg_get(config, "layers_per_block", d.layers_per_block)), heads=int(heads),
                      cross_dim=int(_cfg_get(config, "cross_attention_dim", d.cross_dim)), groups=int(_cfg_get(config, "norm_num_groups", d.groups)),
                      attn_blocks=tuple(t.startswith("CrossAttn") for t in down))


def vae_config_from(config) -> "VAEConfig":
    d = VAEConfig()
    if config is None:
        return d
    return VAEConfig(in_channels=int(_cfg_get(config, "in_channels", d.in_channels)),
                     block_out_channels=tuple(int(c) for c in _cfg_get(config, "block_out_channels", d.block_out_channels)),
                     layers_per_block=int(_cfg_get(config, "layers_per_block", d.layers_per_block)),
                     latent_channels=int(_cfg_get(config, "latent_channels", d.latent_channels)), groups=int(_cfg_get(config, "norm_num_groups", d.groups)),
                     scaling_factor=float(_cfg_get(config, "scaling_factor", d.scaling_factor)))


def _resnet_shapes(sh, pre, cin, cout, temb):
    sh[pre + ".norm1.weight"] = (cin,); sh[pre + ".norm1.bias"] = (cin,)
    sh[pre + ".conv1.weight"] = (cout, cin, 3, 3); sh[pre + ".conv1.bias"] = (cout,)
    if temb:
        sh[pre + ".time_emb_proj.weight"] = (cout, temb); sh[pre + ".time_emb_proj.bias"] = (cout,)
    sh[pre + ".norm2.weight"] = (cout,); sh[pre + ".norm2.bias"] = (cout,)
    sh[pre + ".conv2.weight"] = (cout, cout, 3, 3); sh[pre + ".conv2.bias"] = (cout,)
    if cin != cout:
        sh[pre + ".conv_shortcut.weight"] = (cout, cin, 1, 1); sh[pre + ".conv_shortcut.bias"] = (cout,)


def _transformer_shapes(sh, pre, c, cross):
    sh[pre + ".norm.weight"] = (c,); sh[pre + ".norm.bias"] = (c,)
    sh[pre + ".proj_in.weight"] = (c, c, 1, 1); sh[pre + ".proj_in.bias"] = (c,)
    t = pre + ".transformer_blocks.0"
    for n in ("norm1", "norm2", "norm3"):
        sh["%s.%s.weight" % (t, n)] = (c,); sh["%s.%s.bias" % (t, n)] = (c,)
    for a, kd in (("attn1", c), ("attn2", cross)):
        sh["%s.%s.to_q.weight" % (t, a)] = (c, c)
        sh["%s.%s.to_k.weight" % (t, a)] = (c, kd)
        sh["%s.%s.to_v.weight" % (t, a)] = (c, kd)
        sh["%s.%s.to_out.0.weight" % (t, a)] = (c, c); sh["%s.%s.to_out.0.bias" % (t, a)] = (c,)
    sh[t + ".ff.net.0.proj.weight"] = (8 * c, c); sh[t + ".ff.net.0.proj.bias"] = (8 * c,)
    sh[t + ".ff.net.2.weight"] = (c, 4 * c); sh[t + ".ff.net.2.bias"] = (c,)
    sh[pre + ".proj_out.weight"] = (c, c, 1, 1); sh[pre + ".proj_out.bias"] = (c,)


def _encoder_shapes(sh, cfg: UNetConfig):
    boc = cfg.block_out_channels
    sh["conv_in.weight"] = (boc[0], cfg.in_channels, 3, 3); sh["conv_in.bias"] = (boc[0],)
    sh["time_embedding.linear_1.weight"] = (cfg.temb_dim, boc[0]); sh["time_embedding.linear_1.bias"] = (cfg.temb_dim,)
    sh["time_embedding.linear_2.weight"] = (cfg.temb_dim, cfg.temb_dim); sh["time_embedding.linear_2.bias"] = (cfg.temb_dim,)
    cin = boc[0]
    for i, cout in enumerate(boc):
        for j in range(cfg.layers_per_block):
            _resnet_shapes(sh, "down_blocks.%d.resnets.%d" % (i, j), cin, cout, cfg.temb_dim)
            if cfg.attn_blocks[i]:
                _transformer_shapes(sh, "down_blocks.%d.attentions.%d" % (i, j), cout, cfg.cross_dim)
            cin = cout
        if i != len(boc) - 1:
            sh["down_blocks.%d.downsamplers.0.conv.weight" % i] = (cout, cout, 3, 3)
            sh["down_blocks.%d.downsamplers.0.conv.bias" % i] = (cout,)
    c = boc[-1]
    _resnet_shapes(sh, "mid_block.resnets.0", c, c, cfg.temb_dim)
    _transformer_shapes(sh, "mid_block.attentions.0", c, cfg.cross_dim)
    _resnet_shapes(sh, "mid_block.resnets.1", c, c, cfg.temb_dim)


def _skip_channels(cfg: UNetConfig) -> List[int]:
    boc = cfg.block_out_channels
    ch = [boc[0]]
    for i, cout in enumerate(boc):
        ch += [cout] * cfg.layers_per_block
        if i != len(boc) - 1:
            ch.append(cout)
    return ch


def unet_param_shapes(cfg: UNetConfig) -> "OrderedDict[str, tuple]":
    sh = OrderedDict()
    _encoder_shapes(sh, cfg)
    boc = cfg.block_out_channels
    skips = _skip_channels(cfg)
    rev = list(reversed(boc))
    prev = rev[0]
    for i, cout in enumerate(rev):
        for j in range(cfg.layers_per_block + 1):
            skip = skips.pop()
            _resnet_shapes(sh, "up_blocks.%d.resnets.%d" % (i, j), prev + skip, cout, cfg.temb_dim)
            if list(reversed(cfg.attn_blocks))[i]:
                _transformer_shapes(sh, "up_blocks.%d.attentions.%d" % (i, j), cout, cfg.cross_dim)
            prev = cout
        if i != len(rev) - 1:
            sh["up_blocks.%d.upsamplers.0.conv.weight" % i] = (cout, cout, 3, 3)
            sh["up_blocks.%d.upsamplers.0.conv.bias" % i] = (cout,)
    sh["conv_norm_out.weight"] = (boc[0],); sh["conv_norm_out.bias"] = (boc[0],)
    sh["conv_out.weight"] = (cfg.out_channels, boc[0], 3, 3); sh["conv_out.bias"] = (cfg.out_channels,)
    return sh


def controlnet_param_shapes(cfg: UNetConfig) -> "OrderedDict[str, tuple]":
    sh = OrderedDict()
    _encoder_shapes(sh, cfg)
    cc = cfg.cond_channels
    e = "controlnet_cond_embedding"
    sh[e + ".conv_in.weight"] = (cc[0], cfg.cond_in_channels, 3, 3); sh[e + ".conv_in.bias"] = (cc[0],)
    k = 0
    for i in range(len(cc) - 1):
        sh["%s.blocks.%d.weight" % (e, k)] = (cc[i], cc[i], 3, 3); sh["%s.blocks.%d.bias" % (e, k)] = (cc[i],); k += 1
        sh["%s.blocks.%d.weight" % (e, k)] = (cc[i + 1], cc[i], 3, 3); sh["%s.blocks.%d.bias" % (e, k)] = (cc[i + 1],); k += 1
    sh[e + ".conv_out.weight"] = (cfg.block_out_channels[0], cc[-1], 3, 3); sh[e + ".conv_out.bias"] = (cfg.block_out_channels[0],)
    for k, c in enumerate(_skip_channels(cfg)):
        sh["controlnet_down_blocks.%d.weight" % k] = (c, c, 1, 1); sh["controlnet_down_blocks.%d.bias" % k] = (c,)
    c = cfg.block_out_channels[-1]
    sh["controlnet_mid_block.weight"] = (c, c, 1, 1); sh["controlnet_mid_block.bias"] = (c,)
    return sh


def vae_encoder_param_shapes(cfg: VAEConfig) -> "OrderedDict[str, tuple]":
    sh = OrderedDict()
    boc = cfg.block_out_channels
    sh["encoder.conv_in.weight"] = (boc[0], cfg.in_channels, 3, 3); sh["encoder.conv_in.bias"] = (boc[0],)
    cin = boc[0]
    for i, cout in enumerate(boc):
        for j in range(cfg.layers_per_block):
            _resnet_shapes(sh, "encoder.down_blocks.%d.resnets.%d" % (i, j), cin, cout, 0)
            cin = cout
        if i != len(boc) - 1:
            sh["encoder.down_blocks.%d.downsamplers.0.conv.weight" % i] = (cout, cout, 3, 3)
            sh["encoder.down_blocks.%d.downsamplers.0.conv.bias" % i] = (cout,)
    c = boc[-1]
    _resnet_shapes(sh, "encoder.mid_block.resnets.0", c, c, 0)
    a = "encoder.mid_block.attentions.0"
    sh[a + ".group_norm.weight"] = (c,); sh[a + ".group_norm.bias"] = (c,)
    for n in ("to_q", "to_k", "to_v", "to_out.0"):
        sh["%s.%s.weight" % (a, n)] = (c, c); sh["%s.%s.bias" % (a, n)] = (c,)
    _resnet_shapes(sh, "encoder.mid_block.resnets.1", c, c, 0)
    sh["encoder.conv_norm_out.weight"] = (c,); sh["encoder.conv_norm_out.bias"] = (c,)
    sh["encoder.conv_out.weight"] = (2 * cfg.latent_channels, c, 3, 3); sh["encoder.conv_out.bias"] = (2 * cfg.latent_channels,)
    sh["quant_conv.weight"] = (2 * cfg.latent_channels, 2 * cfg.latent_channels, 1, 1)
    sh["quant_conv.bias"] = (2 * cfg.latent_channels,)
    return sh


def random_state_dict(shapes, seed=0, gain=1.0) -> Dict[str, torch.Tensor]:
    g = torch.Generator().manual_seed(seed)
    sd = OrderedDict()
    for name, shp in shapes.items():
        if "norm" in name and name.endswith("weight") and len(shp) == 1:
            sd[name] = 1.0 + 0.1 * torch.randn(shp, generator=g)
        elif name.endswith("bias"):
            sd[name] = 0.05 * torch.randn(shp, generator=g)
        else:
            fan_in = 1
            for s in shp[1:]:
                fan_in *= s
            sd[name] = torch.randn(shp, generator=g) * (gain / math.sqrt(fan_in))
    return sd


def _pad8(c):
    return (c + 7) // 8 * 8


class Plan:

    def __init__(self, device, dtype="bf16"):
        self.device = device
        self.dtype_name = dtype_name(dtype)
        self.dtype, self.dt = TORCH_DTYPE[self.dtype_name], DT_CODE[self.dtype_name]
        self.esize = 4 if self.dtype_name in ("f32", "f32x") else 2
        self.is_x = self.dtype_name == "f32x"
        self.ops = []
        self.keep = []
        self.tags = []
        self.graph = None
        self.use_graph = True
        self.has_py_ops = False
        self.flops = {}
        self._lib = _lib.lib()
        self.branch = 0
        self._side = {}
        self.scope = ""
        self.labels = []

    def fork(self, b):
        self.ops.append(("fork", 0, b))

    def join(self, b):
        self.ops.append(("fork", b, 0))

    def on_branch(self, b):
        plan = self

        class _Ctx:
            def __enter__(self):
                self.prev, plan.branch = plan.branch, b

            def __exit__(self, *exc):
                plan.branch = self.prev
        return _Ctx()

    def _stream_of(self, b, main):
        if b == 0:
            return main
        if b not in self._side:
            h = ctypes.c_void_p()
            _lib.check(self._lib.dwg_stream_create(ctypes.byref(h)), "dwg_stream_create")
            self._side[b] = h
        return self._side[b]

    def _issue(self, main):
        for op in self.ops:
            if op[0] == "fork":
                rc = self._lib.dwg_stream_fork(self._stream_of(op[1], main), self._stream_of(op[2], main))
            else:
                rc = op[1](self._stream_of(op[0], main))
            if rc:
                raise RuntimeError("plan op failed with DWG error %s" % rc)

    def buf(self, *shape, dtype=None, zero=False):
        dtype = self.dtype if dtype is None else dtype
        zero = zero or os.environ.get("DWG_PLAN_ZERO") == "1"
        t = (torch.zeros if zero else torch.empty)(*shape, device=self.device, dtype=dtype)
        self.keep.append(t)
        self.labels.append((len(self.keep) - 1, self.scope or "op%d" % len(self.ops)))
        self.tags.append((len(self.ops), tuple(shape)))
        return t

    def range_report(self, top=8):
        if not self.is_x:
            return None
        rows = [(i, lab) for (i, lab) in self.labels if self.keep[i].dtype == xfmt.DTYPE and self.keep[i].numel() % 8 == 0 and self.keep[i].numel() > 0
                and self.keep[i].is_contiguous()]
        if not rows:
            return {"tensors": 0, "elements": 0, "saturated": 0, "subnormal": 0, "nonfinite": 0, "max_abs": 0.0, "worst": []}
        cnt = torch.zeros(len(rows), 5, dtype=torch.int64, device=self.device)
        st = ctypes.c_void_p(torch.cuda.current_stream(self.device).cuda_stream)
        for r, (i, _) in enumerate(rows):
            t = self.keep[i]
            _lib.check(self._lib.dwg_xfmt_range_scan(t.numel(), ctypes.c_void_p(t.data_ptr()), ctypes.c_void_p(cnt[r].data_ptr()), st),
                       "dwg_xfmt_range_scan")
        c = cnt.cpu()
        amax = c[:, 3].to(torch.int32).view(torch.float32)
        per = [{"layer": lab, "shape": tuple(self.keep[i].shape), "saturated": int(c[r, 0]), "subnormal": int(c[r, 1]), "nonfinite": int(c[r, 2]),
                "max_abs": float(amax[r])} for r, (i, lab) in enumerate(rows)]
        worst = sorted(per, key=lambda d: (-(d["saturated"] + d["nonfinite"]), -d["max_abs"]))[:top]
        return {"tensors": len(rows), "elements": int(c[:, 4].sum()), "saturated": int(c[:, 0].sum()), "subnormal": int(c[:, 1].sum()),
                "nonfinite": int(c[:, 2].sum()), "max_abs": float(amax.max()), "worst": worst}

    def store(self, dst, src, stage=None):
        if not self.is_x:
            (dst if src.shape == dst.shape else dst[..., :src.shape[-1]]).copy_(src)
            return
        if stage is not None:
            stage[..., :src.shape[-1]].copy_(src)
            src = stage
        elif src.dtype != torch.float32 or not src.is_contiguous():
            src = src.float().contiguous()
        assert src.shape == dst.shape and dst.is_contiguous(), (src.shape, dst.shape)
        _lib.check(self._lib.dwg_xfmt_pack(src.numel(), ctypes.c_void_p(src.data_ptr()), ctypes.c_void_p(dst.data_ptr()),
                                           ctypes.c_void_p(torch.cuda.current_stream(self.device).cuda_stream)), "dwg_xfmt_pack")

    def load(self, t):
        if not (self.is_x and t.dtype == xfmt.DTYPE):
            return t.float()
        out = torch.empty(t.shape, device=t.device, dtype=torch.float32)
        _lib.check(self._lib.dwg_xfmt_unpack(t.numel(), ctypes.c_void_p(t.data_ptr()), ctypes.c_void_p(out.data_ptr()),
                                             ctypes.c_void_p(torch.cuda.current_stream(self.device).cuda_stream)), "dwg_xfmt_unpack")
        return out

    def stage_like(self, buf):
        return torch.zeros(buf.shape, device=self.device, dtype=torch.float32) if self.is_x else None

    def add_gemm(self, desc, allow_split=True):
        if allow_split and desc.batch1 * desc.batch2 == 1 and desc.splitk <= 1 and not desc.accumulate:
            desc.splitk = 0
            need = self._lib.dwg_gemm_workspace_bytes(ctypes.byref(desc))
            if need > 0:
                ws = self.buf(int(need) // 4, dtype=torch.float32)
                desc.workspace, desc.workspace_bytes = ws.data_ptr(), int(need)
            else:
                desc.splitk = 1
        self.keep.append(desc)
        label = desc.name.decode() if desc.name else ("conv_igemm" if desc.conv_enabled else "gemm")
        self.flops[label] = self.flops.get(label, 0.0) + 2.0 * desc.M * desc.N * desc.K * desc.batch1 * desc.batch2
        fn, ref = self._lib.dwg_gemm, ctypes.byref(desc)
        self.ops.append((self.branch, lambda s, fn=fn, ref=ref: fn(ref, s)))

    def add_call(self, fn, *args):
        self.ops.append((self.branch, lambda s, fn=fn, args=args: fn(*args, s)))

    def add_py(self, f):
        self.has_py_ops = True
        self.ops.append((self.branch, lambda s, f=f: (f(), 0)[1]))

    def run_eager(self):
        self._issue(ctypes.c_void_p(torch.cuda.current_stream(self.device).cuda_stream))

    def capture(self):
        if self.graph is not None:
            return
        assert not self.has_py_ops, "plans with Python ops cannot be captured"
        _lib.prof_enable(False)
        self.run_eager()
        torch.cuda.synchronize(self.device)
        self._cap_stream = torch.cuda.Stream(device=self.device)
        s = ctypes.c_void_p(self._cap_stream.cuda_stream)
        _lib.check(self._lib.dwg_graph_begin_capture(s), "dwg_graph_begin_capture")
        try:
            self._issue(s)
        finally:
            h = ctypes.c_void_p()
            rc = self._lib.dwg_graph_end_capture(s, ctypes.byref(h))
        _lib.check(rc, "dwg_graph_end_capture")
        self.graph = h

    def run(self):
        if self.graph is not None and self.use_graph:
            cur = torch.cuda.current_stream(self.device).cuda_stream
            if cur == 0:
                self.run_eager()
                return
            _lib.check(self._lib.dwg_graph_launch(self.graph, ctypes.c_void_p(cur)), "dwg_graph_launch")
        else:
            self.run_eager()

    def run_debug(self):
        s = ctypes.c_void_p(torch.cuda.current_stream(self.device).cuda_stream)
        bufs = [t for t in self.keep if torch.is_tensor(t) and t.is_floating_point()]
        for i, op in enumerate(self.ops):
            rc = 0 if op[0] == "fork" else op[1](s)
            torch.cuda.synchronize()
            bad = [tuple(t.shape) for t in bufs if not torch.isfinite(t.float()).all()]
            if rc or bad:
                return i, rc, bad
        return None


class Weights:

    def __init__(self, sd: Dict[str, torch.Tensor], device, dtype="bf16"):
        self.device = device
        self.sd = sd
        self.cache = {}
        self.wdtype = TORCH_DTYPE[dtype_name(dtype)]
        self.is_x = dtype_name(dtype) == "f32x"

    def _to_dev(self, w):
        if self.is_x:
            a = w.abs()
            r = self.__dict__.setdefault("range", {"elements": 0, "saturated": 0, "subnormal": 0, "max_abs": 0.0})
            r["elements"] += a.numel(); r["saturated"] += int((a >= xfmt.X_MAX).sum()); r["subnormal"] += int(((a < 6.1035e-5) & (a > 0)).sum())
            r["max_abs"] = max(r["max_abs"], float(a.max()) if a.numel() else 0.0)
            return xfmt.pack(w.to(self.device)).contiguous()
        return w.to(self.device, self.wdtype).contiguous()

    def conv(self, name, flip_for_dgrad=False):
        key = (name, flip_for_dgrad)
        if key not in self.cache:
            w = self.sd[name + ".weight"].float()
            if flip_for_dgrad:
                w = w.flip(2, 3).permute(1, 0, 2, 3)
            cout, cin = w.shape[0], w.shape[1]
            wp = torch.zeros(_pad8(cout) if flip_for_dgrad else cout, w.shape[2], w.shape[3], _pad8(cin))
            wp[:cout, :, :, :cin] = w.permute(0, 2, 3, 1)
            self.cache[key] = self._to_dev(wp)
        return self.cache[key]

    def conv_dgrad_s2(self, name, py, px):
        key = ("dgrad_s2", name, py, px)
        if key not in self.cache:
            w = self.sd[name + ".weight"].float()
            kmap = {0: [2, 0], 1: [1]}
            kys, kxs = kmap[py], kmap[px]
            cy, cx = w.shape[0], w.shape[1]
            wp = torch.zeros(_pad8(cx), len(kys), len(kxs), _pad8(cy))
            for ty, ky in enumerate(kys):
                for tx, kx in enumerate(kxs):
                    wp[:cx, ty, tx, :cy] = w[:, :, ky, kx].t()
            self.cache[key] = self._to_dev(wp)
        return self.cache[key]

    def lin(self, *names):
        key = ("lin",) + names
        if key not in self.cache:
            self.cache[key] = self._to_dev(torch.cat([self.sd[n + ".weight"].float().reshape(self.sd[n + ".weight"].shape[0], -1)
                                                      for n in names], 0))
        return self.cache[key]

    def lin_t(self, name):
        key = ("lin_t", name)
        if key not in self.cache:
            w = self.sd[name + ".weight"].float()
            self.cache[key] = self._to_dev(w.reshape(w.shape[0], -1).t().contiguous())
        return self.cache[key]

    def lin_geglu(self, name):
        key = ("geglu", name)
        if key not in self.cache:
            w = self.sd[name + ".weight"].float(); b = self.sd[name + ".bias"].float()
            F = w.shape[0] // 2
            idx = torch.arange(F).view(-1, 32)
            perm = torch.cat([idx, idx + F], dim=1).reshape(-1)
            self.cache[key] = (self._to_dev(w[perm]), b[perm].to(self.device).contiguous())
        return self.cache[key]

    def f32(self, name):
        if name not in self.cache:
            self.cache[name] = self.sd[name].float().to(self.device).contiguous()
        return self.cache[name]

    def bias_cat(self, *names):
        key = ("bias",) + names
        if key not in self.cache:
            self.cache[key] = torch.cat([self.sd[n].float() for n in names], 0).to(self.device).contiguous()
        return self.cache[key]


class Builder:
    def __init__(self, plan: Plan, w: Weights, groups=32, prefix="net"):
        self.p, self.w, self.groups, self.prefix = plan, w, groups, prefix
        self.L = _lib.lib()
        self.full_batch = None

    def _plan_rows(self, b, m):
        return m * self.full_batch // b if self.full_batch and b < self.full_batch and self.full_batch % b == 0 else 0

    def _conv_tag(self, tag, KH, Ho, stride, dil, KW=None):
        if tag:
            return tag
        KW = KH if KW is None else KW
        base = "conv3x3" if KH == 3 else ("conv1x1" if KH * KW == 1 else "conv%dx%d" % (KH, KW))
        return "%s%s_%s_r%d" % (base, "s2" if stride == 2 else ("T" if dil > 1 else ""), self.prefix, Ho)

    def conv(self, x, name, stride=1, pad=1, act=None, residual=None, upsample=1, bias_img=None, out_dtype=None, out_hw=None,
             pad_tl=None, r_batch_bcast=False, weight=None, bias=True, in_dilation=1, tag=None):
        B, H, W, C = x.shape
        self.p.scope = name
        wt = self.w.conv(name) if weight is None else weight
        Cout, KH, KW, Cin = wt.shape
        assert Cin == C, (name, Cin, C)
        Hv, Wv = ((H - 1) * in_dilation + 1) * upsample, ((W - 1) * in_dilation + 1) * upsample
        pt, pl = (pad, pad) if pad_tl is None else pad_tl
        if out_hw is None:
            Ho, Wo = (Hv + 2 * pad - KH) // stride + 1, (Wv + 2 * pad - KW) // stride + 1
        else:
            Ho, Wo = out_hw
        y = self.p.buf(B, Ho, Wo, Cout, dtype=out_dtype)
        b = None
        if bias_img is None and bias:
            b = self.w.f32(name + ".bias")
            if b.numel() < Cout:
                b = None
        conv = (C, H, W, Ho, Wo, KH, KW, stride, pt, pl, in_dilation)
        K = KH * KW * C
        if r_batch_bcast and KH * KW == 1 and stride == 1 and pad == 0 and pad_tl is None and upsample == 1 and in_dilation == 1 and out_hw is None:
            Vr = int(residual.shape[0])
            assert B % Vr == 0 and bias_img is None, (B, Vr)
            Mr = Vr * H * W
            d = gemm.gemm_raw(x, wt, y, Mr, Cout, K, (C, 1), (K, 1), Cout, bias=b, residual=residual, ldr=Cout, act=act, batch=(B // Vr, 1),
                              a_batch=(Mr * C, 0), c_batch=(Mr * Cout, 0), r_batch=(0, 0), name=self._conv_tag(tag, KH, Ho, stride, in_dilation, KW),
                              run=False)
        elif r_batch_bcast:
            Vr = int(residual.shape[0])
            assert B % Vr == 0, (B, Vr)
            d = gemm.gemm_raw(x, wt, y, Ho * Wo, Cout, K, (0, 1), (K, 1), Cout, bias=b, residual=residual, ldr=Cout, act=act,
                              batch=(B // Vr, Vr), a_batch=(Vr * H * W * C, H * W * C), c_batch=(Vr * Ho * Wo * Cout, Ho * Wo * Cout),
                              r_batch=(0, Ho * Wo * Cout), conv=conv,
                              conv_upsample=upsample, name=self._conv_tag(tag, KH, Ho, stride, in_dilation, KW), run=False)
        else:
            kw = {}
            if bias_img is not None:
                kw = dict(bias=bias_img[0], bias_row_div=Ho * Wo, bias_ld=bias_img[1])
            else:
                kw = dict(bias=b)
            d = gemm.gemm_raw(x, wt, y, B * Ho * Wo, Cout, K, (0, 1), (K, 1), Cout, residual=residual,
                              ldr=Cout if residual is not None else 0, act=act, conv=conv, conv_upsample=upsample,
                              name=self._conv_tag(tag, KH, Ho, stride, in_dilation, KW), plan_m=self._plan_rows(B, B * Ho * Wo), run=False, **kw)
        self.p.add_gemm(d)
        return y

    def linear(self, x, wt, bias=None, act=None, residual=None, out_dtype=None, tag="linear"):
        K = x.shape[-1]
        M = x.numel() // K
        N = wt.shape[0]
        Nout = N // 2 if act == "geglu_pair" else N
        y = self.p.buf(*x.shape[:-1], Nout, dtype=out_dtype)
        if residual is not None and residual.numel() != M * Nout:
            R = (M * Nout) // residual.numel()
            Mr = M // R
            assert Mr * R == M and residual.numel() == Mr * Nout and x.is_contiguous(), (M, Nout, tuple(residual.shape))
            d = gemm.gemm_raw(x, wt, y, Mr, N, K, (K, 1), (wt.stride(0), 1), Nout, bias=bias, residual=residual, ldr=Nout, act=act, batch=(R, 1),
                              a_batch=(Mr * K, 0), c_batch=(Mr * Nout, 0), r_batch=(0, 0), name=tag, run=False)
            self.p.add_gemm(d)
            return y
        d = gemm.gemm_raw(x, wt, y, M, N, K, (K, 1), (wt.stride(0), 1), Nout, bias=bias, residual=residual,
                          ldr=Nout if residual is not None else 0, act=act, name=tag, plan_m=self._plan_rows(x.shape[0], M) if x.dim() > 2 else 0,
                          run=False)
        self.p.add_gemm(d)
        return y

    def _gn_ws(self, B):
        need = int(self.L.dwg_groupnorm_workspace_floats(B, self.groups))
        pool = self.p.__dict__.setdefault("_gn_workspace", {})
        ws = pool.get(self.p.branch)
        if ws is None or ws.numel() < need:
            ws = self.p.buf(need, dtype=torch.float32)
            pool[self.p.branch] = ws
        return ws

    def groupnorm(self, x, name, eps, silu, keep_stats=False):
        self.p.scope = name
        B, C = x.shape[0], x.shape[-1]
        HW = x.numel() // (B * C)
        y = self.p.buf(*x.shape)
        stats = self.p.buf(B, self.groups, 2, dtype=torch.float32)
        pp = lambda t: ctypes.c_void_p(t.data_ptr())
        self.p.add_call(self.L.dwg_groupnorm_forward_dt, self.p.dt, B, HW, C, self.groups, pp(x), pp(self.w.f32(name + ".weight")),
                        pp(self.w.f32(name + ".bias")), eps, int(silu), pp(y), pp(stats), pp(self._gn_ws(B)))
        return (y, stats) if keep_stats else y

    def groupnorm_bwd(self, x, dy, stats, name, eps, silu, residual=None):
        B, C = x.shape[0], x.shape[-1]
        HW = x.numel() // (B * C)
        dx = self.p.buf(*x.shape)
        scratch = self.p.buf(B, self.groups, 2, dtype=torch.float32)
        pp = lambda t: ctypes.c_void_p(t.data_ptr())
        self.p.add_call(self.L.dwg_groupnorm_backward_dt, self.p.dt, B, HW, C, self.groups, pp(x), pp(dy), pp(stats),
                        pp(self.w.f32(name + ".weight")), pp(self.w.f32(name + ".bias")), eps, int(silu), pp(dx), pp(scratch),
                        pp(self._gn_ws(B)), pp(residual) if residual is not None else None)
        return dx

    def layernorm(self, x, name):
        self.p.scope = name
        C = x.shape[-1]
        M = x.numel() // C
        y = self.p.buf(*x.shape)
        pp = lambda t: ctypes.c_void_p(t.data_ptr())
        self.p.add_call(self.L.dwg_layernorm_forward_dt, self.p.dt, M, C, pp(x), pp(self.w.f32(name + ".weight")), pp(self.w.f32(name + ".bias")),
                        1e-5, pp(y))
        return y

    def geglu(self, x):
        F2 = x.shape[-1]
        M = x.numel() // F2
        y = self.p.buf(*x.shape[:-1], F2 // 2)
        pp = lambda t: ctypes.c_void_p(t.data_ptr())
        self.p.add_call(self.L.dwg_geglu_forward_dt, self.p.dt, M, F2 // 2, pp(x), pp(y))
        return y

    def _pooled(self, tag, numel, dtype):
        pool = self.p.__dict__.setdefault("_scratch_pool", {})
        key = (tag, self.p.branch, dtype)
        t = pool.get(key)
        if t is None or t.numel() < numel:
            t = pool[key] = self.p.buf(numel, dtype=dtype)
        return t[:numel]

    def attention(self, q, k, v, heads):
        Bq, Nq, HD = q.shape
        B, Nk, d = k.shape[0], k.shape[1], HD // heads
        o = self.p.buf(B, Nq, HD)
        pp = lambda t: ctypes.c_void_p(t.data_ptr())
        if B != Bq:
            R = B // Bq
            assert R * Bq == B and v.shape[0] == B, (B, Bq)
            if self.p.dtype_name == "f32":
                raise NotImplementedError("the exact-f32 plans run attention on dwg_gemm, whose two batch levels are image x head")
            need = int(self.L.dwg_attention_split_workspace_bytes(self.p.dt, B, heads, Nq, Nk, d))
            ws = self.p.buf((need + 3) // 4, dtype=torch.float32) if need > 0 else None
            self.p.add_call(self.L.dwg_attention_forward_pairs_ws, self.p.dt, R, Bq, heads, Nq, Nk, d, pp(q), q.stride(1), q.stride(0), 0,
                            pp(k), k.stride(1), k.stride(0), Bq * k.stride(0), pp(v), v.stride(1), v.stride(0), Bq * v.stride(0),
                            pp(o), o.stride(1), o.stride(0), Bq * o.stride(0), float(d) ** -0.5, pp(ws) if ws is not None else None, need)
            return o
        if self.p.dtype_name == "f32":
            S = self._pooled("attn_S", B * heads * Nq * Nk, torch.float32)
            P = self._pooled("attn_P", B * heads * Nq * Nk, self.p.dtype)
            self.p.add_gemm(gemm.gemm_raw(q, k, S, Nq, Nk, d, (q.stride(1), 1), (k.stride(1), 1), Nk, batch=(B, heads),
                                          a_batch=(q.stride(0), d), b_batch=(k.stride(0), d), c_batch=(heads * Nq * Nk, Nq * Nk),
                                          name="attn_qk", run=False))
            self.p.add_call(self.L.dwg_softmax_rows_forward_dt, self.p.dt, B * heads * Nq, Nk, float(d) ** -0.5, pp(S), Nk, pp(P), Nk)
            self.p.add_gemm(gemm.gemm_raw(P, v, o, Nq, d, Nk, (Nk, 1), (1, v.stride(1)), HD, batch=(B, heads),
                                          a_batch=(heads * Nq * Nk, Nq * Nk), b_batch=(v.stride(0), d), c_batch=(o.stride(0), d),
                                          name="attn_pv", run=False))
            return o
        need = int(self.L.dwg_attention_split_workspace_bytes(self.p.dt, B, heads, Nq, Nk, d))
        if need > 0:
            ws = self.p.buf((need + 3) // 4, dtype=torch.float32)
            self.p.add_call(self.L.dwg_attention_forward_ws, self.p.dt, B, heads, Nq, Nk, d, pp(q), q.stride(1), q.stride(0), pp(k), k.stride(1),
                            k.stride(0), pp(v), v.stride(1), v.stride(0), pp(o), o.stride(1), o.stride(0), float(d) ** -0.5, pp(ws), need)
            return o
        self.p.add_call(self.L.dwg_attention_forward_dt, self.p.dt, B, heads, Nq, Nk, d, pp(q), q.stride(1), q.stride(0), pp(k), k.stride(1),
                        k.stride(0), pp(v), v.stride(1), v.stride(0), pp(o), o.stride(1), o.stride(0), float(d) ** -0.5)
        return o

    def cat(self, a, b):
        Ca, Cb = a.shape[-1], b.shape[-1]
        y = self.p.buf(*a.shape[:-1], Ca + Cb)
        pp = lambda t: ctypes.c_void_p(t.data_ptr())
        k2 = self.p.esize // 2
        if b.shape[0] != a.shape[0]:
            assert a.shape[0] % b.shape[0] == 0 and a.shape[1:-1] == b.shape[1:-1], (tuple(a.shape), tuple(b.shape))
            self.p.add_call(self.L.dwg_concat_channels_bcast, a.numel() // Ca, b.numel() // Cb, Ca * k2, Cb * k2, pp(a), pp(b), pp(y))
            return y
        self.p.add_call(self.L.dwg_concat_channels, a.numel() // Ca, Ca * k2, Cb * k2, pp(a), pp(b), pp(y))
        return y

    def add(self, a, b):
        y = self.p.buf(*a.shape)
        pp = lambda t: ctypes.c_void_p(t.data_ptr())
        self.p.add_call(self.L.dwg_add_dt, self.p.dt, a.numel(), pp(a), pp(b), pp(y))
        return y

    def conv_dgrad_s2(self, dy, name):
        B, Ho, Wo, _ = dy.shape
        subs = []
        for py in (0, 1):
            for px in (0, 1):
                wt = self.w.conv_dgrad_s2(name, py, px)
                subs.append(self.conv(dy, None, weight=wt, bias=False, stride=1, pad_tl=(wt.shape[1] - 1, wt.shape[2] - 1),
                                      out_hw=(Ho, Wo)))
        C = subs[0].shape[-1]
        out = self.p.buf(B, 2 * Ho, 2 * Wo, C)
        pp = lambda t: ctypes.c_void_p(t.data_ptr())
        self.p.add_call(self.L.dwg_interleave2x2, B, Ho, Wo, C * (self.p.esize // 2), pp(subs[0]), pp(subs[1]), pp(subs[2]), pp(subs[3]), pp(out))
        return out

    def transpose(self, x):
        B, R, C = x.shape
        y = self.p.buf(B, C, R)
        pp = lambda t: ctypes.c_void_p(t.data_ptr())
        self.p.add_call(self.L.dwg_transpose_dt, self.p.dt, B, R, C, pp(x), x.stride(1), x.stride(0), pp(y), R, C * R)
        return y

    def cast_bf16(self, x):
        if self.p.dtype_name == "f32":
            return x
        y = self.p.buf(*x.shape)
        pp = lambda t: ctypes.c_void_p(t.data_ptr())
        self.p.add_call(self.L.dwg_cast_f32_to_dt, self.p.dt, x.numel(), pp(x), pp(y))
        return y

    def resnet(self, x, pre, temb_bias, eps=1e-5):
        self.p.scope = pre
        C = x.shape[-1]
        n1 = self.groupnorm(x, pre + ".norm1", eps, True)
        h1 = self.conv(n1, pre + ".conv1", bias_img=temb_bias)
        n2 = self.groupnorm(h1, pre + ".norm2", eps, True)
        Cout = h1.shape[-1]
        sc = x if C == Cout else self.conv(x, pre + ".conv_shortcut", pad=0)
        return self.conv(n2, pre + ".conv2", residual=sc)

    def text_kv(self, text, t):
        batches = self.__dict__.setdefault("_text_kv", {})
        key = text.data_ptr()
        if key not in batches:
            suffix = ".attn2.to_k.weight"
            blocks = sorted(n[:-len(suffix)] for n in self.w.sd if n.endswith(suffix) and self.w.sd[n].shape[1] == text.shape[-1])
            names = []
            for b_ in blocks:
                names += [b_ + ".attn2.to_k", b_ + ".attn2.to_v"]
            out = self.linear(text, self.w.lin(*names), tag="attn_kv")
            offs, o = {}, 0
            for b_ in blocks:
                c = int(self.w.sd[b_ + suffix].shape[0])
                offs[b_] = (o, c); o += 2 * c
            batches[key] = (out, offs, text)
        ent = batches[key]
        if t not in ent[1]:
            return self.linear(text, self.w.lin(t + ".attn2.to_k", t + ".attn2.to_v"), tag="attn_kv")
        o, c = ent[1][t]
        return ent[0][..., o:o + 2 * c]

    def transformer(self, x, pre, text, heads):
        self.p.scope = pre
        B, H, W, C = x.shape
        Bo = text.shape[0]
        n = self.groupnorm(x, pre + ".norm", 1e-6, False)
        h = self.conv(n, pre + ".proj_in", pad=0).view(B, H * W, C)
        t = pre + ".transformer_blocks.0"
        l1 = self.layernorm(h, t + ".norm1")
        qkv = self.linear(l1, self.w.lin(t + ".attn1.to_q", t + ".attn1.to_k", t + ".attn1.to_v"), tag="attn_qkv")
        a = self.attention(qkv[..., :C], qkv[..., C:2 * C], qkv[..., 2 * C:], heads)
        h = self.linear(a, self.w.lin(t + ".attn1.to_out.0"), bias=self.w.f32(t + ".attn1.to_out.0.bias"), residual=h, tag="attn_out")
        l2 = self.layernorm(h, t + ".norm2")
        q = self.linear(l2, self.w.lin(t + ".attn2.to_q"), tag="attn_q")
        kv = self.text_kv(text, t)
        a = self.attention(q, kv[..., :C], kv[..., C:], heads)
        h = self.linear(a, self.w.lin(t + ".attn2.to_out.0"), bias=self.w.f32(t + ".attn2.to_out.0.bias"), residual=h, tag="attn_out")
        l3 = self.layernorm(h, t + ".norm3")
        wg, bg = self.w.lin_geglu(t + ".ff.net.0.proj")
        g = self.linear(l3, wg, bias=bg, act="geglu_pair", tag="ff_in")
        h = self.linear(g, self.w.lin(t + ".ff.net.2"), bias=self.w.f32(t + ".ff.net.2.bias"), residual=h, tag="ff_out")
        return self.conv(h.view(Bo, H, W, C), pre + ".proj_out", pad=0, residual=x, r_batch_bcast=Bo != B)


def timestep_embedding(t: torch.Tensor, dim: int) -> torch.Tensor:
    half = dim // 2
    freqs = torch.exp(-math.log(10000.0) * torch.arange(half, dtype=torch.float32, device=t.device) / half)
    args = t.float()[:, None] * freqs[None]
    return torch.cat([torch.cos(args), torch.sin(args)], dim=-1)


class _TimeEmbed:

    def __init__(self, b: Builder, w: Weights, cfg: UNetConfig, B, resnet_names):
        self.tin = b.p.buf(B, cfg.block_out_channels[0])
        e1 = b.linear(self.tin, w.lin("time_embedding.linear_1"), bias=w.f32("time_embedding.linear_1.bias"), act="silu", tag="temb")
        emb = b.linear(e1, w.lin("time_embedding.linear_2"), bias=w.f32("time_embedding.linear_2.bias"), act="silu", tag="temb")
        names = [n + ".time_emb_proj" for n in resnet_names]
        wt = w.lin(*names)
        bias = w.bias_cat(*[n + ".time_emb_proj.bias" for n in resnet_names]) + w.bias_cat(*[n + ".conv1.bias" for n in resnet_names])
        b.p.keep.append(bias)
        self.all = b.linear(emb, wt, bias=bias, out_dtype=torch.float32, tag="temb_proj")
        self.offsets, off = {}, 0
        for n in resnet_names:
            c = w.sd[n + ".conv1.bias"].numel()
            self.offsets[n] = (off, c); off += c
        self.ld = off

    def bias_for(self, name):
        off, c = self.offsets[name]
        return (self.all[:, off:off + c], self.ld)


def _encoder_resnet_names(cfg: UNetConfig):
    names = []
    for i in range(len(cfg.block_out_channels)):
        for j in range(cfg.layers_per_block):
            names.append("down_blocks.%d.resnets.%d" % (i, j))
    return names + ["mid_block.resnets.0", "mid_block.resnets.1"]


def _build_encoder(b: Builder, cfg: UNetConfig, x, temb: _TimeEmbed, text, hint=None):
    h = b.conv(x, "conv_in", residual=hint, r_batch_bcast=hint is not None)
    skips = [h]
    nb = len(cfg.block_out_channels)
    for i in range(nb):
        for j in range(cfg.layers_per_block):
            pre = "down_blocks.%d.resnets.%d" % (i, j)
            h = b.resnet(h, pre, temb.bias_for(pre))
            if cfg.attn_blocks[i]:
                h = b.transformer(h, "down_blocks.%d.attentions.%d" % (i, j), text, cfg.heads)
            skips.append(h)
        if i != nb - 1:
            h = b.conv(h, "down_blocks.%d.downsamplers.0.conv" % i, stride=2)
            skips.append(h)
    h = b.resnet(h, "mid_block.resnets.0", temb.bias_for("mid_block.resnets.0"))
    h = b.transformer(h, "mid_block.attentions.0", text, cfg.heads)
    h = b.resnet(h, "mid_block.resnets.1", temb.bias_for("mid_block.resnets.1"))
    return skips, h


class DenoiserPlan:

    def __init__(self, cfg: UNetConfig, unet_sd, cn_sd, device, batch=2, latent_hw=64, text_len=77, dtype="bf16", views=1, weights=None,
                 shared_prefix=False):
        self.cfg, self.device, self.B, self.hw, self.views = cfg, device, batch, latent_hw, int(views)
        self.shared_prefix = bool(shared_prefix)
        if self.shared_prefix and batch != 2 * self.views:
            raise ValueError("a shared-prefix plan runs the CFG pair of each view: batch must be 2 * views, got batch %d for %d view(s)" % (batch, self.views))
        if self.shared_prefix and dtype_name(dtype) == "f32":
            raise NotImplementedError("shared_prefix: the exact-f32 plans run attention on dwg_gemm, whose two batch levels are image x head")
        self._temb_table = None
        self.temb_rows = 1001
        assert batch % self.views == 0, (batch, views)
        self.plan = Plan(device, dtype)
        p = self.plan
        self.pre = Plan(device, dtype)
        self._pre_event, self._pre_ready, self._pre_stream = None, False, None
        wu, wc = weights if weights is not None else (Weights(unet_sd, device, dtype), Weights(cn_sd, device, dtype))
        self.weights = (wu, wc)
        bu, bc = Builder(p, wu, cfg.groups, "unet"), Builder(p, wc, cfg.groups, "cnet")
        pu, pc = Builder(self.pre, wu, cfg.groups, "unet"), Builder(self.pre, wc, cfg.groups, "cnet")
        if self.shared_prefix:
            bu.full_batch = bc.full_batch = batch
        B, hw = batch, latent_hw
        self.latents = p.buf(self.views if self.shared_prefix else B, hw, hw, _pad8(cfg.in_channels), zero=True)
        self.text = p.buf(B, text_len, cfg.cross_dim)
        self.cond_scale = 2 ** (len(cfg.cond_channels) - 1)
        self.cond = p.buf(self.views, hw * self.cond_scale, hw * self.cond_scale, _pad8(cfg.cond_in_channels), zero=True)
        self._lat_stage, self._cond_stage = p.stage_like(self.latents), p.stage_like(self.cond)
        up_names = []
        rev_attn = list(reversed(cfg.attn_blocks))
        for i in range(len(cfg.block_out_channels)):
            for j in range(cfg.layers_per_block + 1):
                up_names.append("up_blocks.%d.resnets.%d" % (i, j))
        nb = len(cfg.block_out_channels)

        def decoder(h, skips):
            skips = list(skips)
            for i in range(nb):
                for j in range(cfg.layers_per_block + 1):
                    pre = "up_blocks.%d.resnets.%d" % (i, j)
                    h = bu.resnet(bu.cat(h, skips.pop()), pre, self.temb_u.bias_for(pre))
                    if rev_attn[i]:
                        h = bu.transformer(h, "up_blocks.%d.attentions.%d" % (i, j), self.text, cfg.heads)
                if i != nb - 1:
                    h = bu.conv(h, "up_blocks.%d.upsamplers.0.conv" % i, upsample=2)
            n = bu.groupnorm(h, "conv_norm_out", 1e-5, True)
            return bu.conv(n, "conv_out", out_dtype=torch.float32)

        def zero_convs(cskips, cmid, skips, mid):
            return ([bc.conv(cs, "controlnet_down_blocks.%d" % k, pad=0, residual=skips[k]) for k, cs in enumerate(cskips)],
                    bc.conv(cmid, "controlnet_mid_block", pad=0, residual=mid))

        def hint_embedding(b_):
            e = "controlnet_cond_embedding"
            hnt = b_.conv(self.cond, e + ".conv_in", act="silu")
            for k in range(2 * (len(cfg.cond_channels) - 1)):
                hnt = b_.conv(hnt, "%s.blocks.%d" % (e, k), stride=2 if k % 2 == 1 else 1, act="silu")
            return b_.conv(hnt, e + ".conv_out")
        suffix = ".attn2.to_k"
        first_block = lambda w_: sorted(n[:-len(suffix + ".weight")] for n in w_.sd if n.endswith(suffix + ".weight"))[0]
        self.pre.fork(1)
        with self.pre.on_branch(1):
            self.temb_c = _TimeEmbed(pc, wc, cfg, B, _encoder_resnet_names(cfg))
            hnt = hint_embedding(pc)
            pc.text_kv(self.text, first_block(wc))
        self.temb_u = _TimeEmbed(pu, wu, cfg, B, _encoder_resnet_names(cfg) + up_names)
        pu.text_kv(self.text, first_block(wu))
        self.pre.join(1)
        bu.__dict__["_text_kv"] = pu.__dict__["_text_kv"]
        bc.__dict__["_text_kv"] = pc.__dict__["_text_kv"]
        p.fork(1)
        with p.on_branch(1):
            cskips, cmid = _build_encoder(bc, cfg, self.latents, self.temb_c, self.text, hint=hnt)
        skips, mid = _build_encoder(bu, cfg, self.latents, self.temb_u, self.text)
        p.join(1)
        skips, h = zero_convs(cskips, cmid, skips, mid)
        self.eps = decoder(h, skips)

    def _store_prelude_inputs(self, t, text, cond_nchw):
        p = self.plan
        t = t.reshape(-1)
        if t.numel() not in (1, self.B):
            assert self.B % t.numel() == 0, (self.B, t.numel())
            t = t.repeat(self.B // t.numel())
        if t.dtype == torch.long and t.is_cuda:
            if self._temb_table is None or self._temb_table.shape[0] != self.temb_rows:
                self._temb_table = timestep_embedding(torch.arange(self.temb_rows, device=t.device), self.cfg.block_out_channels[0])
            te = self._temb_table.index_select(0, t.expand(self.B))
        else:
            te = timestep_embedding(t.expand(self.B), self.cfg.block_out_channels[0])
        p.store(self.temb_u.tin, te); p.store(self.temb_c.tin, te)
        p.store(self.text, text)
        if cond_nchw is not None:
            p.store(self.cond, cond_nchw.permute(0, 2, 3, 1), self._cond_stage)

    def prefetch(self, t, text, cond_nchw=None, stream=None):
        dev = self.device
        if stream is None or torch.device(dev).type != "cuda":
            self._store_prelude_inputs(t, text, cond_nchw)
            self.pre.run()
            self._pre_ready, self._pre_event = True, None
            return
        main = torch.cuda.current_stream(dev)
        stream.wait_stream(main)
        with torch.cuda.stream(stream):
            self._store_prelude_inputs(t, text, cond_nchw)
            self.pre.run()
            ev = torch.cuda.Event()
            ev.record(stream)
        for x in (t, text, cond_nchw):
            if torch.is_tensor(x) and x.is_cuda:
                x.record_stream(stream)
        self._pre_ready, self._pre_event = True, ev

    def set_inputs(self, latents_nchw, t=None, text=None, cond_nchw=None):
        if self.shared_prefix and latents_nchw.shape[0] != self.views:
            raise ValueError("a shared-prefix plan takes one latent image per view (%d), got %d" % (self.views, latents_nchw.shape[0]))
        self.plan.store(self.latents, latents_nchw.permute(0, 2, 3, 1), self._lat_stage)
        if not self._pre_ready:
            self._store_prelude_inputs(t, text, cond_nchw)

    def run(self):
        if self._pre_ready:
            if self._pre_event is not None:
                torch.cuda.current_stream(self.device).wait_event(self._pre_event)
        else:
            self.pre.run()
        self._pre_ready, self._pre_event = False, None
        self.plan.run()
        return self.eps.permute(0, 3, 1, 2)


class VAEEncoderPlan:

    def __init__(self, cfg: VAEConfig, sd, device, image_hw=512, dtype="bf16", batch=1, weights=None):
        self.cfg, self.device, self.hw, self.B = cfg, device, image_hw, int(batch)
        self.fwd, self.bwd = Plan(device, dtype), Plan(device, dtype)
        w = weights if weights is not None else Weights(sd, device, dtype)
        self.weights = w
        f, r = Builder(self.fwd, w, cfg.groups, "vaef"), Builder(self.bwd, w, cfg.groups, "vaeb")
        self.x = self.fwd.buf(self.B, image_hw, image_hw, 8, zero=True)
        self._x_stage = self.fwd.stage_like(self.x)
        boc = cfg.block_out_channels
        tape = []

        def conv_f(xin, name, **kw):
            y = f.conv(xin, name, **kw)
            return y

        def resnet_f(xin, pre):
            C = xin.shape[-1]
            n1, s1 = f.groupnorm(xin, pre + ".norm1", 1e-6, True, keep_stats=True)
            h1 = f.conv(n1, pre + ".conv1")
            n2, s2 = f.groupnorm(h1, pre + ".norm2", 1e-6, True, keep_stats=True)
            Cout = h1.shape[-1]
            sc = xin if C == Cout else f.conv(xin, pre + ".conv_shortcut", pad=0)
            out = f.conv(n2, pre + ".conv2", residual=sc)

            def back(dout):
                dn2 = r.conv(dout, None, weight=w.conv(pre + ".conv2", True), bias=False)
                dh1 = r.groupnorm_bwd(h1, dn2, s2, pre + ".norm2", 1e-6, True)
                dn1 = r.conv(dh1, None, weight=w.conv(pre + ".conv1", True), bias=False)
                if C == Cout:
                    return r.groupnorm_bwd(xin, dn1, s1, pre + ".norm1", 1e-6, True, residual=dout)
                dx = r.groupnorm_bwd(xin, dn1, s1, pre + ".norm1", 1e-6, True)
                return r.conv(dout, None, weight=w.conv(pre + ".conv_shortcut", True), pad=0, bias=False, residual=dx)
            tape.append(back)
            return out

        h = f.conv(self.x, "encoder.conv_in")
        tape.append(lambda d: r.conv(d, None, weight=w.conv("encoder.conv_in", True), bias=False))
        for i, cout in enumerate(boc):
            for j in range(cfg.layers_per_block):
                h = resnet_f(h, "encoder.down_blocks.%d.resnets.%d" % (i, j))
            if i != len(boc) - 1:
                name = "encoder.down_blocks.%d.downsamplers.0.conv" % i
                Hin = h.shape[1]
                h = f.conv(h, name, stride=2, pad=0, out_hw=(Hin // 2, Hin // 2))
                tape.append(lambda d, name=name: r.conv_dgrad_s2(d, name))
        h = resnet_f(h, "encoder.mid_block.resnets.0")
        h = self._attention(f, r, w, h, "encoder.mid_block.attentions.0", tape)
        h = resnet_f(h, "encoder.mid_block.resnets.1")
        n, st = f.groupnorm(h, "encoder.conv_norm_out", 1e-6, True, keep_stats=True)
        tape.append(lambda d, h=h, st=st: r.groupnorm_bwd(h, d, st, "encoder.conv_norm_out", 1e-6, True))
        c8 = f.conv(n, "encoder.conv_out")
        tape.append(lambda d: r.conv(d, None, weight=w.conv("encoder.conv_out", True), bias=False))
        self.moments = f.conv(c8, "quant_conv", pad=0, out_dtype=torch.float32)
        tape.append(lambda d: r.conv(d, None, weight=w.conv("quant_conv", True), pad=0, bias=False))
        self.dmoments = self.bwd.buf(*self.moments.shape, zero=True)
        d = self.dmoments
        for back in reversed(tape):
            d = back(d)
        self.dx = d

    @staticmethod
    def _attention(f: Builder, r: Builder, w: Weights, x, pre, tape):
        B, H, W, C = x.shape
        N = H * W
        scale = float(C) ** -0.5
        n, st = f.groupnorm(x, pre + ".group_norm", 1e-6, False, keep_stats=True)
        nt = n.view(B, N, C)
        q = f.linear(nt, w.lin(pre + ".to_q"), bias=w.f32(pre + ".to_q.bias"), tag="vae_qkv")
        k = f.linear(nt, w.lin(pre + ".to_k"), bias=w.f32(pre + ".to_k.bias"), tag="vae_qkv")
        v = f.linear(nt, w.lin(pre + ".to_v"), bias=w.f32(pre + ".to_v.bias"), tag="vae_qkv")
        S = f.p.buf(B, N, N, dtype=torch.float32)
        f.p.add_gemm(gemm.gemm_raw(q, k, S, N, N, C, (C, 1), (C, 1), N, batch=(B, 1), a_batch=(N * C, 0), b_batch=(N * C, 0),
                                   c_batch=(N * N, 0), name="vae_qk", run=False))
        P = f.p.buf(B, N, N)
        pp = lambda t: ctypes.c_void_p(t.data_ptr())
        f.p.add_call(f.L.dwg_softmax_rows_forward_dt, f.p.dt, B * N, N, scale, pp(S), N, pp(P), N)
        o = f.p.buf(B, N, C)
        kc = f.p.esize == 2 or f.p.is_x
        if kc:
            vT = f.transpose(v)
            f.p.add_gemm(gemm.gemm_raw(P, vT, o, N, C, N, (N, 1), (N, 1), C, batch=(B, 1), a_batch=(N * N, 0), b_batch=(N * C, 0),
                                       c_batch=(N * C, 0), name="vae_pv", run=False))
        else:
            f.p.add_gemm(gemm.gemm_raw(P, v, o, N, C, N, (N, 1), (1, C), C, batch=(B, 1), a_batch=(N * N, 0), b_batch=(N * C, 0),
                                       c_batch=(N * C, 0), name="vae_pv", run=False))
        out = f.linear(o, w.lin(pre + ".to_out.0"), bias=w.f32(pre + ".to_out.0.bias"), residual=x.view(B, N, C), tag="vae_out")
        out = out.view(B, H, W, C)

        def back(dout):
            dt = dout.view(B, N, C)
            wo = w.lin(pre + ".to_out.0")
            M = B * N
            bk = dict(batch=(B, 1))
            do = r.p.buf(B, N, C)
            if kc:
                r.p.add_gemm(gemm.gemm_raw(dt, w.lin_t(pre + ".to_out.0"), do, M, C, C, (C, 1), (C, 1), C, name="vae_bwd", run=False))
            else:
                r.p.add_gemm(gemm.gemm_raw(dt, wo, do, M, C, C, (C, 1), (1, C), C, name="vae_bwd", run=False))
            dP = r.p.buf(B, N, N, dtype=torch.float32)
            r.p.add_gemm(gemm.gemm_raw(do, v, dP, N, N, C, (C, 1), (C, 1), N, a_batch=(N * C, 0), b_batch=(N * C, 0), c_batch=(N * N, 0),
                                       name="vae_bwd_dp", run=False, **bk))
            dv = r.p.buf(B, N, C)
            if kc:
                PT, doT = r.transpose(P), r.transpose(do)
                r.p.add_gemm(gemm.gemm_raw(PT, doT, dv, N, C, N, (N, 1), (N, 1), C, a_batch=(N * N, 0), b_batch=(N * C, 0), c_batch=(N * C, 0),
                                           name="vae_bwd_dv", run=False, **bk))
            else:
                r.p.add_gemm(gemm.gemm_raw(P, do, dv, N, C, N, (1, N), (1, C), C, a_batch=(N * N, 0), b_batch=(N * C, 0), c_batch=(N * C, 0),
                                           name="vae_bwd_dv", run=False, **bk))
            dS = r.p.buf(B, N, N)
            r.p.add_call(r.L.dwg_softmax_rows_backward_dt, r.p.dt, B * N, N, scale, pp(P), N, pp(dP), N, pp(dS), N)
            dq = r.p.buf(B, N, C)
            dk = r.p.buf(B, N, C)
            if kc:
                kT, qT, dST = r.transpose(k), r.transpose(q), r.transpose(dS)
                r.p.add_gemm(gemm.gemm_raw(dS, kT, dq, N, C, N, (N, 1), (N, 1), C, a_batch=(N * N, 0), b_batch=(N * C, 0), c_batch=(N * C, 0),
                                           name="vae_bwd_dq", run=False, **bk))
                r.p.add_gemm(gemm.gemm_raw(dST, qT, dk, N, C, N, (N, 1), (N, 1), C, a_batch=(N * N, 0), b_batch=(N * C, 0), c_batch=(N * C, 0),
                                           name="vae_bwd_dk", run=False, **bk))
            else:
                r.p.add_gemm(gemm.gemm_raw(dS, k, dq, N, C, N, (N, 1), (1, C), C, a_batch=(N * N, 0), b_batch=(N * C, 0), c_batch=(N * C, 0),
                                           name="vae_bwd_dq", run=False, **bk))
                r.p.add_gemm(gemm.gemm_raw(dS, q, dk, N, C, N, (1, N), (1, C), C, a_batch=(N * N, 0), b_batch=(N * C, 0), c_batch=(N * C, 0),
                                           name="vae_bwd_dk", run=False, **bk))
            dn = r.p.buf(B, N, C, dtype=torch.float32)
            for i, (g_, wn) in enumerate(((dq, ".to_q"), (dk, ".to_k"), (dv, ".to_v"))):
                if kc:
                    r.p.add_gemm(gemm.gemm_raw(g_, w.lin_t(pre + wn), dn, M, C, C, (C, 1), (C, 1), C, accumulate=i > 0, name="vae_bwd_dn", run=False))
                else:
                    r.p.add_gemm(gemm.gemm_raw(g_, w.lin(pre + wn), dn, M, C, C, (C, 1), (1, C), C, accumulate=i > 0, name="vae_bwd_dn", run=False))
            dnb = r.cast_bf16(dn).view(B, H, W, C)
            dx = r.groupnorm_bwd(x, dnb, st, pre + ".group_norm", 1e-6, False)
            return r.add(dx, dout)
        tape.append(back)
        return out

    def encode(self, image_nchw):
        if self._fused_io(image_nchw):
            img = image_nchw.contiguous()
            _lib.check(self.fwd._lib.dwg_vae_image_pack(self.B, self.hw, self.hw, _lib.ptr(img), _lib.ptr(self.x), self._st()), "dwg_vae_image_pack")
        else:
            self.fwd.store(self.x, (image_nchw * 2.0 - 1.0).permute(0, 2, 3, 1), self._x_stage)
        self.fwd.run()
        return self.moments.permute(0, 3, 1, 2)

    def _st(self):
        return ctypes.c_void_p(torch.cuda.current_stream(self.device).cuda_stream)

    def _fused_io(self, t):
        image = t.dim() == 4 and t.shape[1] == 3 and tuple(t.shape[-2:]) == (self.hw, self.hw)
        grad = t.dim() == 4 and t.shape[1] == 8 and tuple(t.shape[-2:]) == tuple(self.moments.shape[1:3])
        return self.fwd.is_x and t.is_cuda and t.dtype == torch.float32 and (image or grad) and t.shape[0] == self.B

    GRAD_TARGET = 64.0

    def backward(self, dmoments_nchw):
        g = dmoments_nchw
        if self._fused_io(g):
            g = g.detach().contiguous()
            inv = torch.empty(1, device=self.device, dtype=torch.float32)
            h, w_ = int(self.moments.shape[1]), int(self.moments.shape[2])
            _lib.check(self.bwd._lib.dwg_vae_grad_prescale_pack(self.B, h * w_, _lib.ptr(g), self.GRAD_TARGET,
                                                                _lib.ptr(self.dmoments), _lib.ptr(inv), self._st()), "dwg_vae_grad_prescale_pack")
            self.bwd.run()
            out = torch.empty(self.B, 3, self.hw, self.hw, device=self.device, dtype=torch.float32)
            _lib.check(self.bwd._lib.dwg_vae_dx_unpack(self.B, self.hw, self.hw, _lib.ptr(self.dx), _lib.ptr(inv), _lib.ptr(out), self._st()),
                       "dwg_vae_dx_unpack")
            return out
        inv = None
        if self.bwd.dtype_name in ("f32x", "f16"):
            amax = g.detach().abs().amax()
            k = torch.floor(torch.log2(self.GRAD_TARGET / amax.clamp_min(1e-30))).clamp(-60.0, 100.0)
            k = torch.where(amax > 0, k, torch.zeros_like(k))
            g = g * torch.exp2(k)
            inv = torch.exp2(1.0 - k)
        self.bwd.store(self.dmoments, g.permute(0, 2, 3, 1))
        self.bwd.run()
        dx = self.bwd.load(self.dx)[..., :3].permute(0, 3, 1, 2)
        return dx * inv if inv is not None else dx * 2.0
```

### include/dwg_gemm.h

```cpp
#ifndef DWG_GEMM_H
#define DWG_GEMM_H
#include "dwg_types.h"
#ifdef __cplusplus
extern "C" {
#endif


#define DWG_ACT_NONE 0
#define DWG_ACT_RELU 1
#define DWG_ACT_LEAKY_RELU 2
#define DWG_ACT_SILU 3
#define DWG_ACT_GELU 4
#define DWG_ACT_SIGMOID 5
#define DWG_ACT_GEGLU_PAIR 6

typedef struct dwg_gemm_desc {
    const void* A; const void* B; void* C;
    const float* bias;
    const void* residual;
    int32_t M, N, K;
    int64_t a_row_stride, a_k_stride, b_row_stride, b_k_stride, ldc, ldr;
    int32_t batch1, batch2;
    int64_t a_batch1_stride, a_batch2_stride, b_batch1_stride, b_batch2_stride, c_batch1_stride, c_batch2_stride,
        r_batch1_stride, r_batch2_stride;
    int32_t dtype;
    int32_t out_dtype;
    int32_t residual_dtype;
    int32_t act;
    float alpha;
    int32_t bias_per_row;
    int32_t splitk;
    int32_t accumulate;
    int32_t conv_enabled, conv_cin, conv_hin, conv_win, conv_hout, conv_wout, conv_kh, conv_kw, conv_stride, conv_pad_t,
        conv_pad_l, conv_in_dilation;
    int32_t conv_in_upsample;
    const void* A2;
    int32_t conv_cin1;
    int32_t bias_row_div;
    int64_t bias_ld;
    void* workspace;
    size_t workspace_bytes;
    const char* name;
    int32_t plan_m;
} dwg_gemm_desc;

int dwg_gemm(const dwg_gemm_desc* desc, dwg_stream_t stream);

size_t dwg_gemm_workspace_bytes(const dwg_gemm_desc* desc);

#ifdef __cplusplus
}
#endif
#endif
```

Baseline: 41.13.

## Decompose upsample-by-2 3x3 convs into four 2x2 phase convs with strided output

```diff
diff --git a/dreamwaltz-g_amd/csrc/gemm.hip b/dreamwaltz-g_amd/csrc/gemm.hip
--- a/dreamwaltz-g_amd/csrc/gemm.hip
+++ b/dreamwaltz-g_amd/csrc/gemm.hip
@@ -45,6 +45,7 @@
     float* ws;
     int bias_row_div;
     long long bias_ld;
+    int out_phase;
     ConvP conv;
 };
 
@@ -247,8 +248,19 @@
         acc = __builtin_amdgcn_mfma_f32_32x32x2f32(pa[ks * 2], pb[ks * 2], acc, 0, 0, 0);
 }
 
-template <bool LIGHT = false>
-__device__ __forceinline__ void epilogue_store(const GemmP& p, float v, int row, int col, long long coff, long long roff) {
+template <bool REMAP = true>
+__device__ __forceinline__ int out_row(const GemmP& p, int row) {
+    if constexpr (!REMAP) return row;
+    if (p.out_phase == 0) return row;
+    const int hw = p.conv.Hout * p.conv.Wout;
+    const int img = row / hw, rem = row - img * hw;
+    const int i = rem / p.conv.Wout, j = rem - i * p.conv.Wout;
+    return (img * 2 * p.conv.Hout + 2 * i + ((p.out_phase >> 1) & 1)) * 2 * p.conv.Wout + 2 * j + (p.out_phase & 1);
+}
+
+template <bool LIGHT = false, bool REMAP = true>
+__device__ __forceinline__ void epilogue_store(const GemmP& p, float v, int prow, int col, long long coff, long long roff) {
+    const int row = out_row<REMAP>(p, prow);
     const long long ci = coff + (long long)row * p.ldc + col;
     if (p.bias) v += reinterpret_cast<const float*>(p.bias)[p.bias_row_div > 0 ? (long long)(row / p.bias_row_div) * p.bias_ld + col
                                                                              : (p.bias_per_row ? row : col)];
@@ -268,14 +280,15 @@
     return ok;
 }
 
-template <bool LIGHT = false>
-__device__ __forceinline__ void epilogue_store4(const GemmP& p, float (&v)[4], int row, int col, long long coff, long long roff, bool vec_ok) {
+template <bool LIGHT = false, bool REMAP = true>
+__device__ __forceinline__ void epilogue_store4(const GemmP& p, float (&v)[4], int prow, int col, long long coff, long long roff, bool vec_ok) {
     if (!vec_ok || col + 3 >= p.N) {
 #pragma unroll
         for (int e = 0; e < 4; e++)
-            if (col + e < p.N) epilogue_store<LIGHT>(p, v[e], row, col + e, coff, roff);
+            if (col + e < p.N) epilogue_store<LIGHT, REMAP>(p, v[e], prow, col + e, coff, roff);
         return;
     }
+    const int row = out_row<REMAP>(p, prow);
     if (p.bias) {
         const float* b = reinterpret_cast<const float*>(p.bias);
         if (p.bias_row_div > 0) {
@@ -321,7 +334,7 @@
     static constexpr size_t bytes(int npass) { return (size_t)(BM / npass) * LDC * 4; }
 };
 
-template <int BN, int NPASS, int TM, int TN, bool LIGHT, int BM = 128, int NT = 256, typename RowFn>
+template <int BN, int NPASS, int TM, int TN, bool LIGHT, int BM = 128, int NT = 256, bool REMAP = true, typename RowFn>
 __device__ __forceinline__ void tile_epilogue_lds(const GemmP& p, f32x16 (&acc)[TM][TN], float* sC, int n0, int wm, int wn, int lane, int tid,
                                                   int ks_id, long long coff, long long roff, RowFn row_of) {
     constexpr int LDC = EpiLds<BN, BM>::LDC, C4 = BN / 4, PR = BM / NPASS;
@@ -404,14 +417,15 @@
                 const bool slab = p.splitk > 1;
 #pragma unroll 2
                 for (int rl = rl0; rl < PR; rl += RSTEP) {
-                    const int row = row_of(q * PR + rl);
-                    if (row < 0) continue;
+                    const int prow = row_of(q * PR + rl);
+                    if (prow < 0) continue;
                     const float4 a = *reinterpret_cast<const float4*>(sC + rl * LDC + c4 * 4);
                     float v[4] = {a.x * p.alpha, a.y * p.alpha, a.z * p.alpha, a.w * p.alpha};
                     if (slab) {
-                        *reinterpret_cast<float4*>(p.ws + ((long long)ks_id * p.M + row) * p.N + col) = make_float4(v[0], v[1], v[2], v[3]);
+                        *reinterpret_cast<float4*>(p.ws + ((long long)ks_id * p.M + prow) * p.N + col) = make_float4(v[0], v[1], v[2], v[3]);
                         continue;
                     }
+                    const int row = out_row<REMAP>(p, prow);
                     if (col_bias) { v[0] += bc.x; v[1] += bc.y; v[2] += bc.z; v[3] += bc.w; }
                     else if (bias) {
                         const float4 b = *reinterpret_cast<const float4*>(bias + (long long)(row / p.bias_row_div) * p.bias_ld + col);
@@ -468,7 +482,7 @@
                 }
                 continue;
             }
-            epilogue_store4<LIGHT>(p, v, row, col, coff, roff, vec_ok);
+            epilogue_store4<LIGHT, REMAP>(p, v, row, col, coff, roff, vec_ok);
         }
     }
 }
@@ -582,7 +596,7 @@
     }
     constexpr int NPASS = EpiLds<BN>::passes((size_t)2 * (BM + BN) * LDT * sizeof(T));
     static_assert((size_t)2 * (BM + BN) * LDT * sizeof(T) >= EpiLds<BN>::bytes(NPASS), "epilogue staging fits in the operand stages");
-    tile_epilogue_lds<BN, NPASS, TM, TN, false>(p, acc, reinterpret_cast<float*>(smem_raw), n0, wm, wn, lane, tid, ks_id, z1 * p.bC1 + z2 * p.bC2,
+    tile_epilogue_lds<BN, NPASS, TM, TN, false, 128, 256, AMODE == MODE_CONV>(p, acc, reinterpret_cast<float*>(smem_raw), n0, wm, wn, lane, tid, ks_id, z1 * p.bC1 + z2 * p.bC2,
                                          z1 * p.bR1 + z2 * p.bR2, [&](int rl) { const int r = m0 + rl; return r < p.M ? r : -1; });
 }
 
@@ -748,6 +762,8 @@
     static constexpr int WN = BN / 64, WM = (BM == 128 && BN == 64) ? 4 : BM / 64, NW = WM * WN, NT = NW * 64, TM = BM / WM / 32, TN = 2;
 };
 
+constexpr bool glds_remaps(int bm, int bn, int akind) { return akind == 2 || (akind == 1 && bm == 128 && bn == 64); }
+
 template <int BM, int BN, int AKIND, int S>
 __device__ __forceinline__ void gemm_glds_body(const GemmP& p) {
     typedef GldsGeom<BM, BN> Geo;
@@ -910,7 +926,7 @@
 #endif
     constexpr int NPASS = EpiLds<BN, BM>::passes((size_t)S * STAGE);
     static_assert((size_t)S * STAGE >= EpiLds<BN, BM>::bytes(NPASS), "epilogue staging fits in the operand stages");
-    tile_epilogue_lds<BN, NPASS, TM, TN, false, BM, NT>(p, acc, reinterpret_cast<float*>(smem_raw), n0, wm, wn, lane, tid, ks_id, z1 * p.bC1 + z2 * p.bC2,
+    tile_epilogue_lds<BN, NPASS, TM, TN, false, BM, NT, glds_remaps(BM, BN, AKIND)>(p, acc, reinterpret_cast<float*>(smem_raw), n0, wm, wn, lane, tid, ks_id, z1 * p.bC1 + z2 * p.bC2,
                                          z1 * p.bR1 + z2 * p.bR2, [&](int rl) { const int r = m0 + rl; return r < p.M ? r : -1; });
 }
 
@@ -1194,7 +1210,7 @@
 #endif
     constexpr int NPASS = EpiLds<BN, BM>::passes((size_t)2 * PBYTES + NBS * BBYTES);
     static_assert((size_t)2 * PBYTES + NBS * BBYTES >= EpiLds<BN, BM>::bytes(NPASS), "epilogue staging fits in the patch / weight buffers");
-    tile_epilogue_lds<BN, NPASS, TM, TN, !SPLIT, BM, NT>(p, acc, reinterpret_cast<float*>(smem_raw), n0, wm, wn, lane, tid, ks_id, 0, 0, [&](int rr) {
+    tile_epilogue_lds<BN, NPASS, TM, TN, !SPLIT, BM, NT, false>(p, acc, reinterpret_cast<float*>(smem_raw), n0, wm, wn, lane, tid, ks_id, 0, 0, [&](int rr) {
         const int y = y0 + rr / PW, x = x0 + rr % PW;
         return (y < cv.Hout && x < cv.Wout) ? (img * cv.Hout + y) * cv.Wout + x : -1;
     });
@@ -1377,7 +1393,8 @@
     const int patch_min_m = minm ? atoi(minm) : kPatchMinM;
     const bool patch_geom = pl.amode == MODE_CONV && batch_of(d) == 1 && d->conv_kh == 3 && d->conv_kw == 3 && d->conv_stride == 1 &&
                             cv.dil == 1 && cv.up == 1 && d->conv_pad_t == 1 && d->conv_pad_l == 1 && !d->A2 && d->conv_cin % 64 == 0 &&
-                            d->conv_hout == d->conv_hin && d->conv_wout == d->conv_win && d->conv_wout >= 16 && d->conv_hout >= 8;
+                            d->conv_hout == d->conv_hin && d->conv_wout == d->conv_win && d->conv_wout >= 16 && d->conv_hout >= 8 &&
+                            !p.out_phase;
     const int ncc = d->conv_cin / 64;
     if (patch_geom && d->splitk <= 1 && d->conv_hout % 16 == 0 && d->conv_wout % 16 == 0 && (d->N % 128 == 0 || d->N >= 512)) {
         const long long tiles8 = (long long)(d->M / 256) * ((d->N + 127) / 128);
@@ -1414,6 +1431,10 @@
     const bool fast_geom = pl.amode == MODE_CONV && d->conv_cin % 64 == 0 && cv.dil == 1 && cv.up == 1 && d->conv_kh * d->conv_kw <= 32;
     const bool cat_fast = d->A2 && d->conv_cin1 % 64 == 0 && (d->conv_cin - d->conv_cin1) % 64 == 0;
     pl.akind = pl.amode != MODE_CONV ? 0 : (fast_geom && !d->A2 ? 2 : (fast_geom && cat_fast ? 3 : 1));
+    if (p.out_phase && pl.akind != 2) {
+        pl.akind = 1; pl.bn = 64; pl.fam = FAM_GLDS;
+        return DWG_OK;
+    }
     int big_sk = 1;
     const int big_bm = d->splitk <= 1 ? big_tile(d->M, d->N, d->K, &big_sk) : 0;
     if (big_bm) {
@@ -1466,6 +1487,33 @@
 }
 #endif
 
+static bool up2_applies(const dwg_gemm_desc* d) {
+    return d->conv_up2_phase_weights && d->conv_enabled && d->conv_in_upsample == 2 && d->conv_kh == 3 && d->conv_kw == 3 &&
+           d->conv_stride == 1 && d->conv_pad_t == 1 && d->conv_pad_l == 1 && d->conv_in_dilation <= 1 && !d->A2 && d->conv_hin > 0 &&
+           d->conv_win > 0 && d->conv_hout == 2 * d->conv_hin && d->conv_wout == 2 * d->conv_win && d->conv_cin > 0 &&
+           d->K == 9 * d->conv_cin && d->M > 0 && d->M % 4 == 0 && d->batch1 == 1 && d->batch2 == 1 &&
+           (d->conv_out_step == 0 || d->conv_out_step == 1) &&
+           !d->accumulate && d->act != DWG_ACT_GEGLU_PAIR && !(d->splitk > 1 && !d->workspace);
+}
+static dwg_gemm_desc up2_phase(const dwg_gemm_desc* d, int ph) {
+    dwg_gemm_desc q = *d;
+    const int py = ph >> 1, px = ph & 1;
+    const size_t esize = d->dtype == DWG_DTYPE_F32 ? sizeof(float) : sizeof(HT);
+    q.conv_up2_phase_weights = nullptr; q.conv_in_upsample = 1;
+    q.M = d->M / 4; q.K = 4 * d->conv_cin;
+    q.plan_m = d->plan_m > d->M ? d->plan_m / 4 : 0;
+    q.B = reinterpret_cast<const char*>(d->conv_up2_phase_weights) + (size_t)ph * d->N * q.K * esize;
+    q.b_row_stride = q.K; q.b_k_stride = 1;
+    q.conv_kh = q.conv_kw = 2; q.conv_pad_t = 1 - py; q.conv_pad_l = 1 - px;
+    q.conv_hout = d->conv_hin; q.conv_wout = d->conv_win;
+    q.conv_out_step = 2; q.conv_out_oy = py; q.conv_out_ox = px;
+    if (d->workspace) {
+        const size_t quarter = (d->workspace_bytes / 4) & ~(size_t)15;
+        q.workspace = reinterpret_cast<char*>(d->workspace) + (size_t)ph * quarter; q.workspace_bytes = quarter;
+    }
+    return q;
+}
+
 extern "C" {
 
 #if defined(DWG_GEMM_X_TU)
@@ -1483,17 +1531,8 @@
 int dwg_gemm_x(const dwg_gemm_desc* d, dwg_stream_t stream);
 #endif
 
-size_t DWG_GEMM_WS_FN(const dwg_gemm_desc* d) {
-#if !defined(DWG_GEMM_F16_TU) && !defined(DWG_GEMM_X_TU)
-    if (d && d->dtype == DWG_DTYPE_F16) return dwg_gemm_workspace_bytes_f16(d);
-    if (d && d->dtype == DWG_DTYPE_F32X) return dwg_gemm_workspace_bytes_x(d);
-#endif
-#ifdef DWG_GEMM_X_TU
-    dwg_gemm_desc xd;
-    if (!x_physical(d, &xd)) return 0;
-    d = &xd;
-#endif
-    if (!d || d->M <= 0 || d->N <= 0 || !slabs_possible(d)) return 0;
+static size_t workspace_one(const dwg_gemm_desc* d) {
+    if (d->M <= 0 || d->N <= 0 || !slabs_possible(d)) return 0;
     dwg_gemm_desc pd = *d;
     if (d->plan_m > d->M) pd.M = d->plan_m;
     d = &pd;
@@ -1505,18 +1544,31 @@
     return sk > 1 ? (size_t)sk * d->M * d->N * sizeof(float) : 0;
 }
 
-int DWG_GEMM_FN(const dwg_gemm_desc* d, dwg_stream_t stream_) {
+size_t DWG_GEMM_WS_FN(const dwg_gemm_desc* d) {
 #if !defined(DWG_GEMM_F16_TU) && !defined(DWG_GEMM_X_TU)
-    if (d && d->dtype == DWG_DTYPE_F16) return dwg_gemm_f16(d, stream_);
-    if (d && d->dtype == DWG_DTYPE_F32X) return dwg_gemm_x(d, stream_);
+    if (d && d->dtype == DWG_DTYPE_F16) return dwg_gemm_workspace_bytes_f16(d);
+    if (d && d->dtype == DWG_DTYPE_F32X) return dwg_gemm_workspace_bytes_x(d);
 #endif
 #ifdef DWG_GEMM_X_TU
     dwg_gemm_desc xd;
-    if (!x_physical(d, &xd)) return DWG_E_ARG;
+    if (!x_physical(d, &xd)) return 0;
     d = &xd;
 #endif
-    if (!d || !d->A || !d->B || !d->C) return DWG_E_ARG;
+    if (!d) return 0;
+    if (up2_applies(d)) {
+        const dwg_gemm_desc q = up2_phase(d, 0);
+        return 4 * ((workspace_one(&q) + 15) & ~(size_t)15);
+    }
+    return workspace_one(d);
+}
+
+static int gemm_one(const dwg_gemm_desc* d, dwg_stream_t stream_) {
+    if (!d->A || !d->B || !d->C) return DWG_E_ARG;
     if (d->M < 0 || d->N < 0 || d->K < 0 || d->batch1 < 1 || d->batch2 < 1 || d->plan_m < 0) return DWG_E_ARG;
+    if (d->conv_out_step < 0 || d->conv_out_step > 2 || (d->conv_out_oy & ~1) || (d->conv_out_ox & ~1)) return DWG_E_ARG;
+    if (d->conv_out_step == 2 && (!d->conv_enabled || d->conv_hout < 1 || d->conv_wout < 1 || batch_of(d) != 1 || d->accumulate ||
+                                  d->act == DWG_ACT_GEGLU_PAIR || (d->splitk > 1 && !d->workspace) || d->M > 0x7fffffff / 4))
+        return DWG_E_ARG;
     if (d->M == 0 || d->N == 0) return DWG_OK;
     if (d->dtype != DWG_DTYPE_F32 && d->dtype != DWG_DTYPE_HALF) return DWG_E_ARG;
     if (d->splitk > 1 && !d->workspace && (d->out_dtype != DWG_DTYPE_F32 || d->bias || d->residual || d->act)) return DWG_E_ARG;
@@ -1536,7 +1588,7 @@
     p.bias_per_row = d->bias_per_row; p.accumulate = d->accumulate;
     const bool plain1x1 = d->conv_enabled && d->conv_kh == 1 && d->conv_kw == 1 && d->conv_stride == 1 && d->conv_pad_t == 0 &&
                           d->conv_pad_l == 0 && d->conv_in_dilation <= 1 && d->conv_in_upsample <= 1 && !d->A2 && d->conv_hout == d->conv_hin &&
-                          d->conv_wout == d->conv_win && d->K == d->conv_cin && batch_of(d) == 1;
+                          d->conv_wout == d->conv_win && d->K == d->conv_cin && batch_of(d) == 1 && d->conv_out_step != 2;
     if (plain1x1) { p.sam = d->conv_cin; p.sak = 1; }
     p.conv.enabled = d->conv_enabled && !plain1x1;
     p.conv.Cin = d->conv_cin; p.conv.Hin = d->conv_hin; p.conv.Win = d->conv_win; p.conv.Hout = d->conv_hout;
@@ -1545,11 +1597,13 @@
     p.conv.up = d->conv_in_upsample > 1 ? d->conv_in_upsample : 1;
     p.conv.A2 = d->A2; p.conv.cin1 = d->A2 ? d->conv_cin1 : d->conv_cin;
     p.bias_row_div = d->bias_row_div; p.bias_ld = d->bias_ld > 0 ? d->bias_ld : d->N;
+    p.out_phase = d->conv_out_step == 2 ? 4 + 2 * d->conv_out_oy + d->conv_out_ox : 0;
     Plan pl;
     dwg_gemm_desc pd = *d;
     if (d->plan_m > d->M) pd.M = d->plan_m;
     const int rc = make_plan(&pd, p, pl);
     if (rc != DWG_OK) return rc;
+    if (p.out_phase && pl.splitk > 1 && !pl.slabs) return DWG_E_ARG;
     p.splitk = pl.splitk;
     p.ws = pl.slabs ? reinterpret_cast<float*>(d->workspace) : nullptr;
     const int batch = batch_of(d);
@@ -1588,4 +1642,27 @@
     return DWG_OK;
 }
 
-}
+int DWG_GEMM_FN(const dwg_gemm_desc* d, dwg_stream_t stream_) {
+#if !defined(DWG_GEMM_F16_TU) && !defined(DWG_GEMM_X_TU)
+    if (d && d->dtype == DWG_DTYPE_F16) return dwg_gemm_f16(d, stream_);
+    if (d && d->dtype == DWG_DTYPE_F32X) return dwg_gemm_x(d, stream_);
+#endif
+#ifdef DWG_GEMM_X_TU
+    dwg_gemm_desc xd;
+    if (!x_physical(d, &xd)) return DWG_E_ARG;
+    d = &xd;
+#endif
+    if (!d) return DWG_E_ARG;
+    if (up2_applies(d)) {
+        if (!d->A || !d->C) return DWG_E_ARG;
+        for (int ph = 0; ph < 4; ph++) {
+            const dwg_gemm_desc q = up2_phase(d, ph);
+            const int rc = gemm_one(&q, stream_);
+            if (rc != DWG_OK) return rc;
+        }
+        return DWG_OK;
+    }
+    return gemm_one(d, stream_);
+}
+
+}
diff --git a/dreamwaltz-g_amd/gemm.py b/dreamwaltz-g_amd/gemm.py
--- a/dreamwaltz-g_amd/gemm.py
+++ b/dreamwaltz-g_amd/gemm.py
@@ -30,6 +30,8 @@
         ("bias_row_div", ctypes.c_int32), ("bias_ld", ctypes.c_int64),
         ("workspace", ctypes.c_void_p), ("workspace_bytes", ctypes.c_size_t),
         ("name", ctypes.c_char_p), ("plan_m", ctypes.c_int32),
+        ("conv_out_step", ctypes.c_int32), ("conv_out_oy", ctypes.c_int32), ("conv_out_ox", ctypes.c_int32),
+        ("conv_up2_phase_weights", ctypes.c_void_p),
     ]
 
 
@@ -51,7 +53,8 @@
 
 def gemm_raw(A, B, C, M, N, K, a_strides, b_strides, ldc, bias=None, residual=None, ldr=0, act=None, alpha=1.0,
              batch=(1, 1), a_batch=(0, 0), b_batch=(0, 0), c_batch=(0, 0), r_batch=(0, 0), bias_per_row=False, splitk=1,
-             accumulate=False, conv=None, name=None, conv_upsample=1, A2=None, cin1=0, bias_row_div=0, bias_ld=0, plan_m=0, run=True):
+             accumulate=False, conv=None, name=None, conv_upsample=1, A2=None, cin1=0, bias_row_div=0, bias_ld=0, plan_m=0, out_phase=None,
+             up2_weights=None, run=True):
     if not A.is_cuda:
         raise RuntimeError("dreamwaltz_g_amd GEMM runs on the GPU only (HIP kernels)")
     d = GemmDesc()
@@ -87,6 +90,10 @@
     d.bias_ld = bias_ld
     d.name = name.encode() if name else None
     d.plan_m = plan_m
+    if out_phase is not None:
+        d.conv_out_step, d.conv_out_oy, d.conv_out_ox = 2, out_phase[0], out_phase[1]
+    if up2_weights is not None:
+        d.conv_up2_phase_weights = up2_weights.data_ptr()
     if not run:
         return d
     _lib.check(_lib.lib().dwg_gemm(ctypes.byref(d), _stream(A)), "dwg_gemm")
diff --git a/dreamwaltz-g_amd/sd15.py b/dreamwaltz-g_amd/sd15.py
--- a/dreamwaltz-g_amd/sd15.py
+++ b/dreamwaltz-g_amd/sd15.py
@@ -357,7 +357,8 @@
                 desc.splitk = 1
         self.keep.append(desc)
         label = desc.name.decode() if desc.name else ("conv_igemm" if desc.conv_enabled else "gemm")
-        self.flops[label] = self.flops.get(label, 0.0) + 2.0 * desc.M * desc.N * desc.K * desc.batch1 * desc.batch2
+        k = desc.K * 4 // 9 if desc.conv_up2_phase_weights else desc.K
+        self.flops[label] = self.flops.get(label, 0.0) + 2.0 * desc.M * desc.N * k * desc.batch1 * desc.batch2
         fn, ref = self._lib.dwg_gemm, ctypes.byref(desc)
         self.ops.append((self.branch, lambda s, fn=fn, ref=ref: fn(ref, s)))
 
@@ -455,6 +456,21 @@
             self.cache[key] = self._to_dev(wp)
         return self.cache[key]
 
+    def conv_up2(self, name):
+        key = ("up2", name)
+        if key not in self.cache:
+            w = self.sd[name + ".weight"].float()
+            taps = {0: ([0], [1, 2]), 1: ([0, 1], [2])}
+            cout, cin = w.shape[0], w.shape[1]
+            wp = torch.zeros(4, cout, 2, 2, _pad8(cin))
+            for py in (0, 1):
+                for px in (0, 1):
+                    for ty, kys in enumerate(taps[py]):
+                        for tx, kxs in enumerate(taps[px]):
+                            wp[2 * py + px, :, ty, tx, :cin] = sum(w[:, :, ky, kx] for ky in kys for kx in kxs)
+            self.cache[key] = self._to_dev(wp)
+        return self.cache[key]
+
     def lin(self, *names):
         key = ("lin",) + names
         if key not in self.cache:
@@ -491,6 +507,9 @@
         return self.cache[key]
 
 
+UP2_MIN_ROWS = 512
+
+
 class Builder:
     def __init__(self, plan: Plan, w: Weights, groups=32, prefix="net"):
         self.p, self.w, self.groups, self.prefix = plan, w, groups, prefix
@@ -508,11 +527,19 @@
         return "%s%s_%s_r%d" % (base, "s2" if stride == 2 else ("T" if dil > 1 else ""), self.prefix, Ho)
 
     def conv(self, x, name, stride=1, pad=1, act=None, residual=None, upsample=1, bias_img=None, out_dtype=None, out_hw=None,
-             pad_tl=None, r_batch_bcast=False, weight=None, bias=True, in_dilation=1, tag=None):
+             pad_tl=None, r_batch_bcast=False, weight=None, bias=True, in_dilation=1, tag=None, out=None, out_phase=None):
         B, H, W, C = x.shape
         self.p.scope = name
-        wt = self.w.conv(name) if weight is None else weight
-        Cout, KH, KW, Cin = wt.shape
+        up2 = None
+        if (upsample == 2 and weight is None and stride == 1 and pad == 1 and pad_tl is None and out_hw is None and in_dilation == 1
+                and not r_batch_bcast and tuple(self.w.sd[name + ".weight"].shape[2:]) == (3, 3)
+                and (self._plan_rows(B, B * H * W) or B * H * W) >= UP2_MIN_ROWS):
+            up2 = self.w.conv_up2(name)
+            Cout, KH, KW, Cin = up2.shape[1], 3, 3, up2.shape[4]
+            wt = up2
+        else:
+            wt = self.w.conv(name) if weight is None else weight
+            Cout, KH, KW, Cin = wt.shape
         assert Cin == C, (name, Cin, C)
         Hv, Wv = ((H - 1) * in_dilation + 1) * upsample, ((W - 1) * in_dilation + 1) * upsample
         pt, pl = (pad, pad) if pad_tl is None else pad_tl
@@ -520,7 +547,11 @@
             Ho, Wo = (Hv + 2 * pad - KH) // stride + 1, (Wv + 2 * pad - KW) // stride + 1
         else:
             Ho, Wo = out_hw
-        y = self.p.buf(B, Ho, Wo, Cout, dtype=out_dtype)
+        if out is None:
+            y = self.p.buf(B, Ho, Wo, Cout, dtype=out_dtype)
+        else:
+            assert out_phase is not None and tuple(out.shape) == (B, 2 * Ho, 2 * Wo, Cout) and not r_batch_bcast, (name, tuple(out.shape))
+            y = out
         b = None
         if bias_img is None and bias:
             b = self.w.f32(name + ".bias")
@@ -550,7 +581,8 @@
                 kw = dict(bias=b)
             d = gemm.gemm_raw(x, wt, y, B * Ho * Wo, Cout, K, (0, 1), (K, 1), Cout, residual=residual,
                               ldr=Cout if residual is not None else 0, act=act, conv=conv, conv_upsample=upsample,
-                              name=self._conv_tag(tag, KH, Ho, stride, in_dilation, KW), plan_m=self._plan_rows(B, B * Ho * Wo), run=False, **kw)
+                              name=self._conv_tag(tag, KH, Ho, stride, in_dilation, KW), plan_m=self._plan_rows(B, B * Ho * Wo),
+                              out_phase=out_phase if out is not None else None, up2_weights=up2, run=False, **kw)
         self.p.add_gemm(d)
         return y
 
@@ -688,16 +720,12 @@
 
     def conv_dgrad_s2(self, dy, name):
         B, Ho, Wo, _ = dy.shape
-        subs = []
+        out = self.p.buf(B, 2 * Ho, 2 * Wo, self.w.conv_dgrad_s2(name, 0, 0).shape[0])
         for py in (0, 1):
             for px in (0, 1):
                 wt = self.w.conv_dgrad_s2(name, py, px)
-                subs.append(self.conv(dy, None, weight=wt, bias=False, stride=1, pad_tl=(wt.shape[1] - 1, wt.shape[2] - 1),
-                                      out_hw=(Ho, Wo)))
-        C = subs[0].shape[-1]
-        out = self.p.buf(B, 2 * Ho, 2 * Wo, C)
-        pp = lambda t: ctypes.c_void_p(t.data_ptr())
-        self.p.add_call(self.L.dwg_interleave2x2, B, Ho, Wo, C * (self.p.esize // 2), pp(subs[0]), pp(subs[1]), pp(subs[2]), pp(subs[3]), pp(out))
+                self.conv(dy, None, weight=wt, bias=False, stride=1, pad_tl=(wt.shape[1] - 1, wt.shape[2] - 1), out_hw=(Ho, Wo),
+                          out=out, out_phase=(py, px))
         return out
 
     def transpose(self, x):
diff --git a/include/dwg_gemm.h b/include/dwg_gemm.h
--- a/include/dwg_gemm.h
+++ b/include/dwg_gemm.h
@@ -42,6 +42,9 @@
     size_t workspace_bytes;
     const char* name;
     int32_t plan_m;
+    int32_t conv_out_step;
+    int32_t conv_out_oy, conv_out_ox;
+    const void* conv_up2_phase_weights;
 } dwg_gemm_desc;
 
 int dwg_gemm(const dwg_gemm_desc* desc, dwg_stream_t stream);
```

Result: no change. 41.52 (median of 6 runs) (+0.9%).
